# goodgodgd/xpt-mde-2021

Hardware: AMD Instinct MI355X
Metric: train images/sec (5-frame 128x416 snippets) (higher is better)
Workload: dtype bf16; 1 GPU; DepthNet(NASNetMobile)+PoseNetImproved train step, KITTI-raw-shaped 5x128x416 snippets, batch 8/GPU, mono L1+SSIM+smoothness, 4 scales; global_batch=8, per_gpu_batch=8, mode=graph, parallelism=dp1, ranks=1

## Files before the change

### include/xpt_hip.h

```cpp
#ifndef XPT_HIP_H_
#define XPT_HIP_H_

#include <stddef.h>
#include <stdint.h>

#ifdef __cplusplus
extern "C" {
#endif

#define XPT_OK 0
#define XPT_ERR_NULL (-1)
#define XPT_ERR_SHAPE (-2)
#define XPT_ERR_ARG (-3)
#define XPT_ERR_WORKSPACE (-4)
#define XPT_ERR_LAUNCH (-5)

#define XPT_PHOTO_L1 0
#define XPT_PHOTO_L2 1
#define XPT_PHOTO_SSIM 2

int xpt_abi_version(void);
const char* xpt_build_arch(void);

int xpt_pose_rvec2matr_fwd(const float* pose, float* T, int M, void* stream);
int xpt_pose_rvec2matr_bwd(const float* pose, const float* dT, float* dpose, int M, void* stream);

int xpt_resize_down_fwd(const float* img, float* out, int M, int H, int W, int C, int scale, void* stream);
int xpt_image_pyramids(const float* image5d, int B, int S, int H, int W, int njobs, const int* first_frame,
                       const int* nframes, const int* scale, float* const* out, void* stream);

int xpt_warp_fwd(const float* src, const float* depth, const float* T, const float* K, float* synth,
                 int B, int N, int h, int w, float scale, void* stream);
size_t xpt_warp_bwd_workspace_floats(int B, int N, int h, int w);
int xpt_warp_bwd(const float* src, const float* depth, const float* T, const float* K, const float* dsynth,
                 float* ddepth, float* dT, float* workspace, size_t workspace_floats,
                 int B, int N, int h, int w, float scale, void* stream);

int xpt_bilinear_fwd(const float* image, const float* coords, const float* valid_mask, float* out,
                     int B, int N, int h, int w, int C, int ncoord, void* stream);
int xpt_bilinear_bwd(const float* image, const float* coords, const float* valid_mask, const float* dout,
                     float* dcoords, int B, int N, int h, int w, int C, int ncoord, void* stream);

size_t xpt_photo_workspace_floats(int B, int N, int h, int w);
int xpt_photo_fwd(int method, const float* synth, const float* target, float* map, float* loss,
                  float* workspace, size_t workspace_floats, int B, int N, int h, int w, void* stream);
int xpt_photo_bwd(int method, const float* synth, const float* target, const float* gloss, const float* gmap,
                  float* dsynth, float* workspace, size_t workspace_floats, int B, int N, int h, int w,
                  void* stream);

int xpt_photo_fused_tune(int fwd_min_waves, int bwd_min_waves, int min_rows);
int xpt_photo_fused_variant(int pipelined);
size_t xpt_photo_fused_workspace_floats(int B, int N, int h, int w);
int xpt_photo_fused_fwd(const float* src, const float* depth, const float* T, const float* K, const float* target,
                        float* synth, float* loss_l1, float* loss_ssim, float* workspace, size_t workspace_floats,
                        int B, int N, int h, int w, float scale, void* stream);
int xpt_photo_fused_bwd(const float* src, const float* depth, const float* T, const float* K, const float* target,
                        const float* g_l1, const float* g_ssim, float* ddepth, float* dT, float* workspace,
                        size_t workspace_floats, int B, int N, int h, int w, float scale, void* stream);

int xpt_photo_fused_ms_fwd(int nscales, const float* const* src, const float* const* depth, const float* T, const float* K,
                           const float* const* target, float* losses, float* workspace, size_t workspace_floats,
                           int B, int N, const int* h, const int* w, const float* scale, void* stream);

int xpt_photo_fused_ms_bwd(int nscales, const float* const* src, const float* const* depth, const float* T, const float* K,
                           const float* const* target, const float* const* g_l1, const float* const* g_ssim,
                           float* const* ddepth, float* dT, float* workspace, size_t workspace_floats, int B, int N,
                           const int* h, const int* w, const float* scale, void* stream);

int xpt_photo_march_tune(int fwd_min_waves, int bwd_min_waves, int min_rows);
int xpt_photo_march_plan(int bwd_variant, int rows_s0, int rows_s1, int rows_s2, int rows_s3);
int xpt_photo_march_ms_fwd(int nscales, const float* const* src, const float* const* depth, const float* T, const float* K,
                           const float* const* target, float* losses, float* workspace, size_t workspace_floats,
                           int B, int N, const int* h, const int* w, const float* scale, void* stream);
int xpt_photo_march_ms_fwdbwd(int nscales, const float* const* src, const float* const* depth, const float* T, const float* K,
                              const float* const* target, const float* const* g_l1, const float* const* g_ssim,
                              float* losses, float* const* ddepth, float* dT, float* workspace, size_t workspace_floats,
                              int B, int N, const int* h, const int* w, const float* scale, void* stream);
int xpt_photo_march_ms_bwd(int nscales, const float* const* src, const float* const* depth, const float* T, const float* K,
                           const float* const* target, const float* const* g_l1, const float* const* g_ssim,
                           float* const* ddepth, float* dT, float* workspace, size_t workspace_floats, int B, int N,
                           const int* h, const int* w, const float* scale, void* stream);

size_t xpt_smooth_workspace_floats(int B, int h, int w);
int xpt_smooth_fwd(const float* disp, const float* image, float* loss, float* workspace, size_t workspace_floats,
                   int B, int h, int w, float grad_factor, int input_is_depth, void* stream);
int xpt_smooth_bwd(const float* disp, const float* image, const float* gloss, float* dinput,
                   int B, int h, int w, float grad_factor, int input_is_depth, void* stream);
int xpt_smooth_ms_fwd(int nscales, const float* const* disp, const float* const* image, float* losses,
                      float* workspace, size_t workspace_floats, int B, const int* h, const int* w, float grad_factor,
                      int input_is_depth, void* stream);
int xpt_smooth_ms_bwd(int nscales, const float* const* disp, const float* const* image, const float* const* gloss,
                      float* const* dinput, int B, const int* h, const int* w, float grad_factor, int input_is_depth,
                      void* stream);

int xpt_merge_total_fwd(int n, const float* const* terms, const float* c, const float* amat, float* total,
                        float* by_type, int batch, int types, void* stream);
int xpt_merge_total_bwd(int n, const float* c, const float* g_total, float* grads, int batch, void* stream);

int xpt_adam_step(float* param, float* grad, float* m, float* v, long long n, const float* step, float lr,
                  float beta1, float beta2, float eps, float grad_scale, int zero_grad, void* shadow_bf16,
                  void* stream);
int xpt_sgd_step(float* param, float* grad, long long n, float lr, float grad_scale, int zero_grad, void* shadow_bf16,
                 void* stream);

typedef struct xpt_loss_scale_state {
  float scale;
  float inv_scale;
  int found_inf;
  int good_steps;
  int skipped;
  int reserved[3];
} xpt_loss_scale_state;
int xpt_grad_nonfinite(const float* g, long long n, void* state, void* stream);
int xpt_loss_scale_update(void* state, int growth_steps, void* stream);
int xpt_adam_step_dyn(float* param, float* grad, float* m, float* v, long long n, const float* step, float lr,
                      float beta1, float beta2, float eps, float grad_scale, int zero_grad, void* shadow_bf16,
                      const void* state, void* stream);
int xpt_sgd_step_dyn(float* param, float* grad, long long n, float lr, float grad_scale, int zero_grad, void* shadow_bf16,
                     const void* state, void* stream);

int xpt_dwconv_fwd(const void* x, const float* w, void* y, int B, int H, int W, int C, int k, int stride, int pad_t,
                   int pad_l, int OH, int OW, int relu_in, int dtype, void* stream);
int xpt_dwconv_bwd_data(const void* x, const float* w, const void* dy, void* dx, int B, int H, int W, int C, int k,
                        int stride, int pad_t, int pad_l, int OH, int OW, int relu_in, int dtype, void* stream);
int xpt_dwconv_tune(int wrw_groups);
int xpt_set_xcd_affinity(int on);
int xpt_half_format(void);
size_t xpt_dwconv_bwd_weight_workspace_floats(int B, int OH, int OW, int C, int k);
int xpt_dwconv_bwd_weight(const void* x, const void* dy, float* dw, float* workspace, size_t workspace_floats,
                          int B, int H, int W, int C, int k, int stride, int pad_t, int pad_l, int OH, int OW,
                          int relu_in, int dtype, void* stream);

int xpt_affine_act_fwd(const void* x, const float* gamma, const float* beta, const float* mean, const float* var,
                       float eps, const void* residual, void* y, long long rows, int C, float slope, int relu_in,
                       int dtype, void* stream);
size_t xpt_affine_act_bwd_workspace_floats(long long rows, int C);
int xpt_affine_act_bwd(const void* x, const void* y, const void* dy, long long dy_pitch, const float* gamma,
                       const float* beta, const float* mean, const float* var, float eps, void* dx, float* dbeta,
                       float* dgamma, float* workspace, size_t workspace_floats, long long rows, int C, float slope,
                       int relu_in, int dtype, void* stream);

int xpt_conv1x1_bwd_weight_tune(int waves, int pairs_per_wave, int max_blocks, int max_partial_kib);
int xpt_conv1x1_bwd_weight_defer_cap(int mib);
size_t xpt_conv1x1_bwd_weight_workspace_floats(long long M, int cout, int cin);
int xpt_conv1x1_bwd_weight_counters(long long M, int cout, int cin);
int xpt_conv1x1_bwd_weight(const void* dy, const void* x, float* dw, float* workspace, size_t workspace_floats,
                           unsigned* counters, int n_counters, long long M, int cout, int cin, long long pitch_dy,
                           long long pitch_x, void* stream);

int xpt_pwconv_tune(int ksplit_min_cin, int ksplit_max_tiles);
int xpt_pwconv_bn_fwd(const void* x, const void* w, const float* gamma, const float* beta, const float* mean,
                      const float* var, float eps, const void* residual, void* ypre, void* y, long long M, int cin,
                      int cout, long long pitch_x, void* stream);

typedef struct xpt_conv_pack_job {
  const float* src;
  void* fwd;
  void* bwd;
  long long sn, sc, sh, sw;
  int N, T, KW, C, Cp, Np;
  long long first_block;
} xpt_conv_pack_job;
int xpt_conv_pack_job_bytes(void);
int xpt_conv_pack_weights(const void* jobs, int njobs, long long nblocks, void* stream);
int xpt_conv2d_tune(int plan);
int xpt_conv2d_fwd(const void* x, const void* w, const float* bias, void* y, int B, int PH, int PW, int C,
                   long long xpitch, int N, int KH, int KW, int stride, int pad_t, int pad_l, int OH, int OW,
                   long long ypitch, int upsample, float slope, void* stream);
int xpt_conv2d_bwd_data(const void* g, const void* wb, void* dx, int B, int OH, int OW, int Np, long long gpitch,
                        int C, int KH, int KW, int stride, int pad_t, int pad_l, int IH, int IW, long long dxpitch,
                        int fold2x2, void* stream);
int xpt_conv2d_splitk_tune(int enable, int force_split, int min_k, int max_pixels);
size_t xpt_conv2d_splitk_workspace_floats(long long pixels, int out_channels, int red_channels, int taps, int stride);
int xpt_conv2d_fwd_splitk(const void* x, const void* w, const float* bias, void* y, int B, int PH, int PW, int C,
                          long long xpitch, int N, int KH, int KW, int pad_t, int pad_l, int OH, int OW, long long ypitch,
                          int upsample, float slope, float* workspace, size_t workspace_floats, void* stream);
int xpt_conv2d_bwd_data_splitk(const void* g, const void* wb, void* dx, int B, int OH, int OW, int Np, long long gpitch,
                               int C, int KH, int KW, int pad_t, int pad_l, int IH, int IW, long long dxpitch, int fold2x2,
                               float* workspace, size_t workspace_floats, void* stream);
int xpt_conv2d_stream_tune(int enable, int min_tiles, int wgs_per_cu, int max_lds_kib);
int xpt_conv2d_stream_serves(int B, int OH, int OW, int out_channels, int red_channels, int KH, int KW, int stride,
                             int upsample_or_fold);
int xpt_conv2d_fwd_stream(const void* x, const void* w, const float* bias, void* y, int B, int PH, int PW, int C,
                          long long xpitch, int N, int pad_t, int pad_l, int OH, int OW, long long ypitch, int upsample,
                          float slope, void* stream);
int xpt_conv2d_fwd_stream_k5s2(const void* x, const void* w, const float* bias, void* y, int B, int PH, int PW, int C,
                               long long xpitch, int N, int pad_t, int pad_l, int OH, int OW, long long ypitch, float slope,
                               void* stream);
int xpt_conv2d_bwd_data_stream(const void* g, const void* wb, void* dx, int B, int OH, int OW, int Np, long long gpitch, int C,
                               int pad_t, int pad_l, int IH, int IW, long long dxpitch, int fold2x2, void* stream);
int xpt_conv2d_bwd_weight_tune(int max_partial_mib, int target_blocks);
int xpt_conv2d_bwd_weight_splits(int B, int C, int N, int KH, int KW, int stride, int OH, int OW);
int xpt_conv2d_bwd_weight_partials(const void* g, const void* x, float* partials, size_t partial_floats, int B, int PH,
                                   int PW, int C, int Cr, long long xpitch, int N, long long gpitch, int KH, int KW,
                                   int stride, int pad_t, int pad_l, int OH, int OW, int upsample, void* stream);
int xpt_restack_bf16(const float* image5d, void* out, int B, int S, int H, int W, int Cp, void* stream);

int xpt_headconv_tune(int passes, int max_blocks);
int xpt_headconv_bwd_blocks(int B, int H, int W, int C);
int xpt_headconv_fwd(const void* x, long long xpitch, const float* w, const float* bias, float* pre, int B, int H, int W,
                     int C, void* stream);
int xpt_headconv_bwd(const void* x, long long xpitch, const float* w, const float* g, void* dx, float* partials,
                     size_t partial_floats, int B, int H, int W, int C, void* stream);
int xpt_headconv_bwd_add(const void* x, long long xpitch, const float* w, const float* g, const void* addend,
                         long long addend_pitch, void* dx, float* partials, size_t partial_floats, int B, int H, int W, int C,
                         void* stream);

int xpt_depth_head_fwd(const float* x, float* depth, float* disp, long long n, void* stream);
int xpt_depth_head_bwd(const float* x, const float* g_depth, const float* g_disp, float* gx, long long n, void* stream);
int xpt_depth_head_ms_fwd(int nscales, const float* const* x, float* const* depth, float* const* disp, const long long* n,
                          void* stream);
int xpt_depth_head_ms_bwd(int nscales, const float* const* x, const float* const* g_depth, const float* const* g_disp,
                          float* const* gx, const long long* n, void* stream);

int xpt_global_avgpool_fwd(const void* x, float* y, int B, int HW, int C, int dtype, void* stream);
int xpt_global_avgpool_bwd(const float* g, void* dx, int B, int HW, int C, int dtype, void* stream);

int xpt_upsample2x_fwd(const float* src, void* out, long long M, int h, int w, int dtype, void* stream);
int xpt_upsample2x_bwd(const void* g, long long g_pitch, float* dsrc, long long M, int h, int w, int dtype, void* stream);
int xpt_upsample2x_bwd_add(const void* g, long long g_pitch, const float* addend, float* dsrc, long long M, int h, int w, int dtype,
                           void* stream);

int xpt_corr_cost_channels(int max_disp, int stride2);
int xpt_corr_cost_fwd(const void* left, const void* right, void* out, int B, int H, int W, int C, int max_disp,
                      int stride2, int dtype, void* stream);
int xpt_corr_cost_bwd(const void* left, const void* right, const void* gout, void* dleft, void* dright, int B, int H,
                      int W, int C, int max_disp, int stride2, int dtype, void* stream);

int xpt_avgpool3_same(const void* in, long long in_pitch, void* out, int B, int H, int W, int C, float scale, int adjoint,
                      int dtype, void* stream);

int xpt_pwconv_bn_multi_fwd(int n, const void* const* x, const void* const* w, const float* const* gamma,
                            const float* const* beta, const float* const* mean, const float* const* var, float eps,
                            const void* const* residual, void* const* ypre, void* const* y, long long M, int cin, int cout,
                            long long pitch_x, void* stream);
int xpt_pwconv_bn_multi_fwd_sib(int n, const void* const* x, const void* const* w, const float* const* gamma,
                                const float* const* beta, const float* const* mean, const float* const* var, float eps,
                                const void* const* residual, void* const* ypre, void* const* y, const void* const* sib_x,
                                const void* const* sib_w, const float* const* sib_gamma, const float* const* sib_beta,
                                const float* const* sib_mean, const float* const* sib_var, void* const* sib_ypre,
                                long long M, int cin, int cout, long long pitch_x, long long pitch_y, void* stream);

int xpt_multi_copy(const void* const* src, void* const* dst, const long long* bytes, int n, void* stream);

int xpt_concat_channels(const void* const* inputs, const long long* pitches, const int* channels, int n, void* out,
                        long long rows, int Ct, void* stream);

int xpt_sum_rows(const void* const* inputs, const long long* pitches, int n, void* out, long long rows, int C, int dtype,
                 void* stream);

int xpt_cell_tail_fwd(int nslices, const int* nterms, const void* const* src, const long long* pitch, const int* pooled,
                      const float* scale, void* out, long long out_pitch, int B, int H, int W, int F, int dtype,
                      void* stream);

int xpt_cell_tail_bwd(int ngrads, const void* const* grads, const long long* gpitch, const void* out, long long out_pitch,
                      void* gm, int nslices, int ndense, void* const* dense_out, const int* bterms, const int* slice,
                      const int* pooled, const float* scale, int B, int H, int W, int F, int dtype, void* stream);

int xpt_adjust_gather(const void* in, long long in_pitch, void* out, int B, int H, int W, int C, int dtype, void* stream);
int xpt_adjust_scatter(const void* d1, long long pitch1, const void* d2, long long pitch2, void* out, int B, int H, int W,
                       int C, int dtype, void* stream);

int xpt_pool_pair_fwd(const void* in, long long in_pitch, void* mp, void* ap, void* arg, int B, int H, int W, int C, int OH,
                      int OW, int pad_t, int pad_l, int dtype, void* stream);
int xpt_pool_pair_bwd(const void* gmp, long long pitch_m, const void* gap, long long pitch_a, const void* arg, void* dh, int B,
                      int H, int W, int C, int OH, int OW, int pad_t, int pad_l, int dtype, void* stream);
int xpt_pool_pair_bwd2(const void* gmp, long long pitch_m, const void* gmp2, long long pitch_m2, const void* gap, long long pitch_a,
                       const void* arg, void* dh, int B, int H, int W, int C, int OH, int OW, int pad_t, int pad_l, int dtype,
                       void* stream);

int xpt_augment(const float* u, float* params, const float* img0, float* img0_out, const float* img1, float* img1_out,
                int n_img, const float* depth, float* depth_out, int n_depth, const float* K0, float* K0_out, const float* K1,
                float* K1_out, int B, const float* pose0, float* pose0_out, const float* pose1, float* pose1_out, int n_pose,
                const float* stereo, float* stereo_out, int H, int W, float p_crop, float p_flip, float p_jit,
                float half_crop, void* stream);
int xpt_augment_pin(const float* pin);

int xpt_stem_input(const float* image, long long batch_stride, void* out, int B, int H, int W, void* stream);

int xpt_depth_metric(const float* pred, const float* gt, float* per_sample, int B, int h, int w, int r0, int r1, int c0,
                     int c1, float min_depth, float max_depth, void* stream);

int xpt_pose_metric(const float* pred, const float* truth, float* out, int B, int N, void* stream);

typedef struct xpt_reduce_job {
  float* dst;
  long long n;
  int nseg;
  int split_waves;
  const float* src[4];
  long long stride[4];
  int nsplit[4];
} xpt_reduce_job;
int xpt_reduce_job_bytes(void);
int xpt_reduce_partials(const void* jobs, const void* blockmap, int nblocks, void* stream);
int xpt_affine_act_bwd_blocks(long long rows, int C);
int xpt_affine_act_bwd_partials(const void* x, const void* y, const void* dy, long long dy_pitch, const float* gamma,
                                const float* beta, const float* mean, const float* var, float eps, void* dx,
                                float* partials, size_t partial_floats, long long rows, int C, float slope, int relu_in,
                                int dtype, void* stream);
int xpt_dwconv_bwd_weight_chunks(int B, int OH, int OW, int C, int k, int stride);
int xpt_dwconv_bwd_weight_partials(const void* x, const void* dy, float* partials, size_t partial_floats, int B, int H,
                                   int W, int C, int k, int stride, int pad_t, int pad_l, int OH, int OW, int relu_in,
                                   int dtype, void* stream);
int xpt_dwconv_bwd_both(const void* x, const float* w, const void* dy, void* dx, float* partials, size_t partial_floats,
                        int B, int H, int W, int C, int k, int stride, int pad_t, int pad_l, int OH, int OW, int relu_in,
                        int dtype, void* stream);
int xpt_conv1x1_bn_multi_bwd_partials(int n, const void* const* dy, const long long* pitch_dy, const void* const* ypre,
                                      const void* const* x, const float* const* gamma, const float* const* var,
                                      const float* const* mean, float eps, void* const* g_out, float* const* w_partials,
                                      float* const* bn_partials, size_t w_partial_floats, size_t bn_partial_floats,
                                      long long M, int cout, int cin, long long pitch_x, void* stream);
int xpt_conv1x1_bwd_fused(const void* dy, const void* x, const void* w, void* dx, float* partials,
                          size_t partial_floats, long long M, int cout, int cin, long long pitch_dy, long long pitch_x,
                          void* stream);
int xpt_conv1x1_bn_bwd_fused(const void* dy, const void* dy2, const void* dy3, const void* ypre, const void* x,
                             const void* w, const float* gamma, const float* var, const float* mean, float eps, void* dx,
                             float* w_partials, size_t w_partial_floats, float* bn_partials, size_t bn_partial_floats,
                             long long M, int cout, int cin, long long pitch_dy, long long pitch_dy2, long long pitch_dy3,
                             long long pitch_x, void* stream);
int xpt_conv1x1_bn_multi_bwd_fused(int n, const void* const* dy, const long long* pitch_dy, const void* const* ypre,
                                   const void* const* x, const void* const* w, const float* const* gamma,
                                   const float* const* var, const float* const* mean, float eps, void* const* dx,
                                   float* const* w_partials, float* const* bn_partials, size_t w_partial_floats,
                                   size_t bn_partial_floats, long long M, int cout, int cin, long long pitch_x,
                                   void* stream);
int xpt_conv1x1_bn_multi_bwd_fused_fan(int n, const void* const* dy, const long long* pitch_dy, const void* const* dy2,
                                       const long long* pitch_dy2, const void* const* dy3, const long long* pitch_dy3,
                                       const void* const* ypre, const void* const* x, const void* const* w,
                                       const float* const* gamma, const float* const* var, const float* const* mean,
                                       float eps, void* const* dx, float* const* w_partials, float* const* bn_partials,
                                       size_t w_partial_floats, size_t bn_partial_floats, long long M, int cout, int cin,
                                       long long pitch_x, void* stream);
int xpt_dwconv_multi_fwd(const void* const* x, const float* const* w, void* const* y, const int* k, const int* pad_t,
                         const int* pad_l, int n, int B, int H, int W, int C, int stride, int OH, int OW, int relu_in,
                         int dtype, void* stream);
int xpt_dwconv_multi_bwd(const void* const* xin, void* const* dxin, int n_inputs, const void* const* dy,
                         const float* const* w, float* const* partials, const int* k, const int* pad_t,
                         const int* pad_l, const int* input_of, int n, int B, int H, int W, int C, int stride, int OH,
                         int OW, int relu_in, int dtype, void* stream);
int xpt_conv1x1_bwd_weight_splits(long long M, int cout, int cin);
int xpt_conv1x1_bn_bwd_partials(const void* dy, const void* ypre, const void* x, const float* gamma, const float* var,
                                const float* mean, float eps, void* g_out, float* w_partials, size_t w_partial_floats,
                                float* bn_partials, size_t bn_partial_floats, long long M, int cout, int cin,
                                long long pitch_dy, long long pitch_x, void* stream);
int xpt_conv1x1_bn_bwd_partials_sum(const void* dy, const void* dy2, const void* dy3, const void* ypre, const void* x,
                                    const float* gamma, const float* var, const float* mean, float eps, void* g_out,
                                    float* w_partials, size_t w_partial_floats, float* bn_partials,
                                    size_t bn_partial_floats, long long M, int cout, int cin, long long pitch_dy,
                                    long long pitch_dy2, long long pitch_dy3, long long pitch_x, void* stream);
int xpt_conv1x1_bwd_weight_partials(const void* dy, const void* x, float* partials, size_t partial_floats, long long M,
                                    int cout, int cin, long long pitch_dy, long long pitch_x, void* stream);

uint32_t xpt_crc32c(const void* data, size_t nbytes);
long long xpt_tfrecord_index(const void* shard, size_t nbytes, int verify_crc, unsigned long long* payload_off,
                             unsigned long long* payload_len, unsigned int* payload_crc, long long max_records);
int xpt_tfrecord_decode(const void* payload, size_t nbytes, unsigned int stored_crc, int verify_crc, int nkeys,
                        const char* const* keys, void* const* dst, const size_t* dst_bytes);

int xpt_sepconv_bn_multi_fwd(int n, const void* const* x, const float* const* wdw, const void* const* wpw,
                             const float* const* gamma, const float* const* beta, const float* const* mean,
                             const float* const* var, const int* k, void* const* ydw, void* const* ypre,
                             const void* const* x_b, const float* const* wdw_b, const void* const* wpw_b,
                             const float* const* gamma_b, const float* const* beta_b, const float* const* mean_b,
                             const float* const* var_b, const int* k_b, void* const* ydw_b, void* const* ypre_b,
                             void* const* yb, const void* const* residual, void* const* y, float eps, int B, int H, int W,
                             int C, int cout, void* stream);

int xpt_dwconv_bn_relu6_fwd(const void* x, const float* w, const float* gamma, const float* beta, const float* mean,
                            const float* var, float eps, void* y, int B, int H, int W, int C, int stride, int pad_t, int pad_l,
                            int OH, int OW, int act_in, void* stream);
int xpt_dwconv_bn_relu6_tune(int fwd_outputs);
int xpt_dwconv_bn_relu6_fwd_outputs(int B, int OH, int OW, int C);
int xpt_dwconv_bn_relu6_bwd_chunks(int B, int OH, int OW, int C);
int xpt_dwconv_bn_relu6_bwd(const void* x, const void* y, const void* dy, long long dy_pitch, const float* w,
                            const float* gamma, const float* mean, const float* var, float eps, void* dx, float* partials,
                            size_t partial_floats, int B, int H, int W, int C, int stride, int pad_t, int pad_l, int OH, int OW,
                            int act_in, void* stream);

int xpt_graph_node_census(void* hip_graph, int* counts);

#ifdef __cplusplus
}
#endif
#endif
```

### xpt_mde_2021_amd/csrc/xpt_common.h

```cpp
#pragma once
#include <hip/hip_runtime.h>
#include <stdint.h>

#include "../../include/xpt_hip.h"

#define XPT_WAVE 64

#include <hip/hip_bf16.h>
#include <hip/hip_fp16.h>
#ifdef XPT_HALF_F16
typedef _Float16 xpt_h16;
typedef __half xpt_half_t;
#define XPT_MFMA_32X32X16(a, b, c) __builtin_amdgcn_mfma_f32_32x32x16_f16(a, b, c, 0, 0, 0)
#else
typedef __bf16 xpt_h16;
typedef __hip_bfloat16 xpt_half_t;
#define XPT_MFMA_32X32X16(a, b, c) __builtin_amdgcn_mfma_f32_32x32x16_bf16(a, b, c, 0, 0, 0)
#endif
typedef xpt_h16 xpt_h16x8 __attribute__((ext_vector_type(8)));
#ifdef __HIPCC__
__device__ __forceinline__ float xpt_h2f(unsigned short u) {
#ifdef XPT_HALF_F16
  return (float)__builtin_bit_cast(_Float16, u);
#else
  return __uint_as_float(((unsigned)u) << 16);
#endif
}
__device__ __forceinline__ float xpt_h2f_lo(unsigned w) {
#ifdef XPT_HALF_F16
  return (float)__builtin_bit_cast(_Float16, (unsigned short)(w & 0xffffu));
#else
  return __uint_as_float(w << 16);
#endif
}
__device__ __forceinline__ float xpt_h2f_hi(unsigned w) {
#ifdef XPT_HALF_F16
  return (float)__builtin_bit_cast(_Float16, (unsigned short)(w >> 16));
#else
  return __uint_as_float(w & 0xffff0000u);
#endif
}
__device__ __forceinline__ unsigned short xpt_f2h(float f) {
  return __builtin_bit_cast(unsigned short, (xpt_h16)f);
}
__device__ __forceinline__ unsigned short xpt_f2h_sw(float f) {
#ifdef XPT_HALF_F16
  return xpt_f2h(f);
#else
  unsigned u = __float_as_uint(f);
  u += 0x7fffu + ((u >> 16) & 1u);
  return (unsigned short)(u >> 16);
#endif
}
__device__ __forceinline__ float xpt_half2float(xpt_half_t h) {
#ifdef XPT_HALF_F16
  return __half2float(h);
#else
  return __bfloat162float(h);
#endif
}
__device__ __forceinline__ xpt_half_t xpt_float2half(float f) {
#ifdef XPT_HALF_F16
  return __float2half(f);
#else
  return __float2bfloat16(f);
#endif
}
#endif

#define XPT_CHECK_PTR(p) \
  do {                   \
    if ((p) == nullptr) return XPT_ERR_NULL; \
  } while (0)

static inline int xpt_launch_status() { return hipGetLastError() == hipSuccess ? XPT_OK : XPT_ERR_LAUNCH; }
#define XPT_BEGIN_LAUNCH() (void)hipGetLastError()

__device__ __forceinline__ unsigned xpt_divmod(unsigned n, unsigned d, unsigned& rem) {
  const float inv = __builtin_amdgcn_rcpf((float)d);
  unsigned q = (unsigned)((float)n * inv);
  int r = (int)(n - q * d);
  q += (unsigned)(int)((float)r * inv);
  r = (int)(n - q * d);
  if (r < 0) { --q; r += (int)d; }
  if (r < 0) { --q; r += (int)d; }
  if (r >= (int)d) { ++q; r -= (int)d; }
  if (r >= (int)d) { ++q; r -= (int)d; }
  rem = (unsigned)r;
  return q;
}
__device__ __forceinline__ void xpt_split4(unsigned idx, int n0, int n1, int n2, int& i0, int& i1, int& i2, int& i3) {
  unsigned r0, r1, r2;
  unsigned q = xpt_divmod(idx, (unsigned)n0, r0);
  q = xpt_divmod(q, (unsigned)n1, r1);
  q = xpt_divmod(q, (unsigned)n2, r2);
  i0 = (int)r0; i1 = (int)r1; i2 = (int)r2; i3 = (int)q;
}

namespace xpt {

struct Cam {
  float k[9];
  float ki[9];
};

__device__ inline Cam load_cam(const float* __restrict__ K, float scale) {
  Cam c;
#pragma unroll
  for (int i = 0; i < 6; ++i) c.k[i] = K[i] / scale;
  c.k[6] = 0.f;
  c.k[7] = 0.f;
  c.k[8] = 1.f;
  const float a = c.k[0], b = c.k[1], cc = c.k[2], d = c.k[3], e = c.k[4], f = c.k[5], g = c.k[6], h = c.k[7],
              i = c.k[8];
  const float A = e * i - f * h, Bc = -(d * i - f * g), Cc = d * h - e * g;
  const float det = a * A + b * Bc + cc * Cc;
  const float r = 1.0f / det;
  c.ki[0] = A * r;
  c.ki[1] = -(b * i - cc * h) * r;
  c.ki[2] = (b * f - cc * e) * r;
  c.ki[3] = Bc * r;
  c.ki[4] = (a * i - cc * g) * r;
  c.ki[5] = -(a * f - cc * d) * r;
  c.ki[6] = Cc * r;
  c.ki[7] = -(a * h - b * g) * r;
  c.ki[8] = (a * e - b * d) * r;
  return c;
}

struct Pose {
  float r[9];
  float t[3];
};

__device__ inline Pose load_pose(const float* __restrict__ T) {
  Pose p;
#pragma unroll
  for (int i = 0; i < 3; ++i) {
    p.r[3 * i + 0] = T[4 * i + 0];
    p.r[3 * i + 1] = T[4 * i + 1];
    p.r[3 * i + 2] = T[4 * i + 2];
    p.t[i] = T[4 * i + 3];
  }
  return p;
}

struct Warp {
  float X[3];
  float ray[3];
  float up, vp;
  float zinv;
};

__device__ inline void backproject(const Cam& c, float u, float v, float d, Warp& w) {
#pragma unroll
  for (int i = 0; i < 3; ++i) {
    w.ray[i] = c.ki[3 * i + 0] * u + c.ki[3 * i + 1] * v + c.ki[3 * i + 2];
    w.X[i] = w.ray[i] * d;
  }
}

__device__ inline void project(const Cam& c, const Pose& p, Warp& w) {
  float Xs[3], q[3];
#pragma unroll
  for (int i = 0; i < 3; ++i) Xs[i] = p.r[3 * i + 0] * w.X[0] + p.r[3 * i + 1] * w.X[1] + p.r[3 * i + 2] * w.X[2] + p.t[i];
#pragma unroll
  for (int i = 0; i < 3; ++i) q[i] = c.k[3 * i + 0] * Xs[0] + c.k[3 * i + 1] * Xs[1] + c.k[3 * i + 2] * Xs[2];
  const float z = q[2] + 1e-10f;
  w.zinv = 1.0f / z;
  w.up = q[0] / z;
  w.vp = q[1] / z;
}

struct Taps {
  int uf, uc, vf, vc;
  float wuf, wuc, wvf, wvc;
  float mask;
};

__device__ inline float clampf(float x, float lo, float hi) { return fminf(fmaxf(x, lo), hi); }

__device__ inline Taps make_taps(float u, float v, int h, int w, bool extra_valid) {
  Taps t;
  const float fu = floorf(u), fv = floorf(v);
  const float ufc = clampf(fu, 0.f, (float)(w - 1));
  const float ucc = clampf(fu + 1.f, 0.f, (float)(w - 1));
  const float vfc = clampf(fv, 0.f, (float)(h - 1));
  const float vcc = clampf(fv + 1.f, 0.f, (float)(h - 1));
  const bool ok = (ufc + 1.f == ucc) && (vfc + 1.f == vcc) && extra_valid;
  t.mask = ok ? 1.f : 0.f;
  t.uf = ok ? (int)ufc : 0;
  t.uc = ok ? (int)ucc : 0;
  t.vf = ok ? (int)vfc : 0;
  t.vc = ok ? (int)vcc : 0;
  t.wuf = ok ? (ucc - u) : 0.f;
  t.wuc = ok ? (u - ufc) : 0.f;
  t.wvf = ok ? (vcc - v) : 0.f;
  t.wvc = ok ? (v - vfc) : 0.f;
  return t;
}

__device__ inline float wave_sum(float v) {
#pragma unroll
  for (int off = 32; off > 0; off >>= 1) v += __shfl_down(v, off, 64);
  return v;
}

__device__ inline float block_sum(float v, float* red) {
  const int lane = threadIdx.x & 63, wid = threadIdx.x >> 6, nw = (blockDim.x + 63) >> 6;
  v = wave_sum(v);
  __syncthreads();
  if (lane == 0) red[wid] = v;
  __syncthreads();
  float s = 0.f;
  if (threadIdx.x == 0) {
    for (int i = 0; i < nw; ++i) s += red[i];
  }
  return s;
}

template <int NV>
__device__ inline void block_sum_n(float (&v)[NV], float* red) {
  const int lane = threadIdx.x & 63, wid = threadIdx.x >> 6, nw = (blockDim.x + 63) >> 6;
#pragma unroll
  for (int i = 0; i < NV; ++i) v[i] = wave_sum(v[i]);
  __syncthreads();
  if (lane == 0) {
#pragma unroll
    for (int i = 0; i < NV; ++i) red[wid * NV + i] = v[i];
  }
  __syncthreads();
  if (threadIdx.x == 0) {
#pragma unroll
    for (int i = 0; i < NV; ++i) {
      float s = 0.f;
      for (int k = 0; k < nw; ++k) s += red[k * NV + i];
      v[i] = s;
    }
  }
}

}

extern int g_xpt_xcd_affinity;
#ifdef __HIPCC__
__device__ __forceinline__ void xpt_xcd_remap(bool on, unsigned& bx, unsigned& by, unsigned gx, unsigned gy) {
  if (!on) return;
  const unsigned lin = bx + gx * by, total = gx * gy;
  const unsigned u = (lin & 7u) * (total >> 3) + (lin >> 3);
  by = u / gx;
  bx = u - by * gx;
}
#endif
inline bool xpt_xcd_ok(unsigned long long total) { return g_xpt_xcd_affinity != 0 && total % 8 == 0 && total >= 64; }

inline unsigned xpt_xcd_pad(unsigned long long n) { return (unsigned)((n + 7) & ~7ull); }
inline unsigned xpt_magic(unsigned d) { return d <= 1 ? 0u : (unsigned)((0x100000000ull + d - 1) / d); }
#ifdef __HIPCC__
__device__ __forceinline__ unsigned xpt_fastdiv(unsigned n, unsigned m) { return m ? __umulhi(n, m) : n; }
#endif

struct XcdSweep {
  unsigned grid, units, per;
  int on;
#ifdef __HIPCC__
  __device__ __forceinline__ bool range(unsigned x, long long total, long long& begin, long long& end) const;
#endif
};
inline XcdSweep xpt_xcd_sweep(long long total, long long max_units, int threads = 256) {
  XcdSweep s;
  long long units = (total + threads - 1) / threads;
  if (units > max_units) units = max_units;
  if (units < 1) units = 1;
  s.per = (unsigned)(((total + units - 1) / units + threads - 1) / threads * threads);
  s.units = (unsigned)((total + s.per - 1) / s.per);
  if (s.units < 1) s.units = 1;
  s.on = g_xpt_xcd_affinity;
  s.grid = s.on ? xpt_xcd_pad(s.units) : s.units;
  return s;
}
#ifdef __HIPCC__
__device__ __forceinline__ bool xpt_xcd_unit(bool on, unsigned x, unsigned n, unsigned& u) {
  if (!on) {
    u = x;
    return x < n;
  }
  const unsigned k = x & 7u, q = x >> 3;
  const unsigned lo = (k * n) >> 3, hi = ((k + 1u) * n) >> 3;
  u = lo + q;
  return u < hi;
}
inline unsigned xpt_xcd_two_class_grid(int on, unsigned nA, unsigned LA, unsigned nB, unsigned LB) {
  return on ? nA * xpt_xcd_pad(LA) + nB * xpt_xcd_pad(LB) : nA * LA + nB * LB;
}
__device__ __forceinline__ bool xpt_xcd_two_class(bool on, unsigned x, unsigned nA, unsigned LA, unsigned nB, unsigned LB,
                                                  unsigned& vb) {
  if (!on) {
    vb = x;
    return true;
  }
  const unsigned a8 = nA * ((LA + 7u) & ~7u);
  const bool first = x < a8;
  const unsigned L = first ? LA : LB, lin = first ? x : x - a8;
  const unsigned c8 = (L + 7u) >> 3, k = lin & 7u, q = lin >> 3;
  unsigned local;
  const unsigned seg = xpt_divmod(q, c8, local);
  const unsigned lo = (k * L) >> 3, hi = ((k + 1u) * L) >> 3;
  vb = (first ? 0u : nA * LA) + seg * L + lo + local;
  return lo + local < hi;
}
__device__ __forceinline__ void xpt_chunk_range(unsigned blk, unsigned nblocks, long long total, long long& begin, long long& end) {
  unsigned rem_;
  const unsigned per = (xpt_divmod((unsigned)total + nblocks - 1u, nblocks, rem_) + 255u) & ~255u;
  begin = (long long)blk * per;
  end = begin + per < total ? begin + per : total;
}
__device__ __forceinline__ bool XcdSweep::range(unsigned x, long long total, long long& begin, long long& end) const {
  unsigned u;
  if (!xpt_xcd_unit(on != 0, x, units, u)) return false;
  begin = (long long)u * per;
  end = begin + per < total ? begin + per : total;
  return true;
}
#endif
```

### xpt_mde_2021_amd/csrc/xpt_conv_wgrad.hip

```cpp
#include "xpt_common.h"

namespace {

typedef float f32x16 __attribute__((ext_vector_type(16)));
typedef xpt_h16x8 bf16x8;
typedef short s16x4 __attribute__((ext_vector_type(4)));
typedef short s16x8 __attribute__((ext_vector_type(8)));
typedef unsigned int u32x4 __attribute__((ext_vector_type(4)));

constexpr int WGRAD_MAXCH = 12;

struct WgradArgs {
  const unsigned short* g;
  const unsigned short* x;
  float* part;
  long long gpitch, xpitch, gbytes, xbytes;
  int B, PH, PW, shift, Hlim, Wlim;
  int C, Cr, N, KH, KW, stride, pad_t, pad_l, OH, OW;
  int R, CB, nseg, nrb, units, nsplit;
  int WN, WC, WT;
  int dbg;
};

__device__ inline bf16x8 tr_pair(const char* lds, unsigned off0, unsigned off1) {
  typedef s16x4 __attribute__((address_space(3))) * lds_ptr;
  const s16x4 lo = __builtin_amdgcn_ds_read_tr16_b64_v4i16((lds_ptr)(lds + off0));
  const s16x4 hi = __builtin_amdgcn_ds_read_tr16_b64_v4i16((lds_ptr)(lds + off1));
  s16x8 v;
  v[0] = lo[0]; v[1] = lo[1]; v[2] = lo[2]; v[3] = lo[3];
  v[4] = hi[0]; v[5] = hi[1]; v[6] = hi[2]; v[7] = hi[3];
  return __builtin_bit_cast(bf16x8, v);
}

template <int MAXCH>
struct WgradChunks {
  int row[MAXCH], col[MAXCH];
  unsigned chb[MAXCH];
};

constexpr unsigned WG_OOB = 0x40000000u;

template <int MAXCH>
__device__ __forceinline__ void wgrad_chunks(const WgradArgs& a, int tid, int n0, int c0, int TNB, int TCB, int Wt,
                                             int gi, int gchunks, int xchunks, WgradChunks<MAXCH>& w) {
  const int lg = __builtin_ctz((unsigned)(TNB >> 3)), lx = __builtin_ctz((unsigned)(TCB >> 3));
  const float inv_cb = 1.f / (float)a.CB, inv_wt = 1.f / (float)Wt;
#pragma unroll
  for (int i = 0; i < MAXCH; ++i) {
    if (i < gi) {
      const int ck = tid + 256 * i;
      const int gc8 = ck & ((1 << lg) - 1), gpix = ck >> lg;
      const int gr = (int)(((float)gpix + 0.5f) * inv_cb);
      w.row[i] = gr;
      w.col[i] = gpix - gr * a.CB;
      const int n = n0 + 8 * gc8;
      w.chb[i] = (ck < gchunks && n < a.N) ? (unsigned)n * 2u : WG_OOB;
    } else {
      const int cx = tid + 256 * (i - gi);
      const int xc8 = cx & ((1 << lx) - 1), xpix = cx >> lx;
      const int xr = (int)(((float)xpix + 0.5f) * inv_wt);
      w.row[i] = xr;
      w.col[i] = xpix - xr * Wt;
      const int c = c0 + 8 * xc8;
      w.chb[i] = (cx < xchunks && c < a.C) ? (unsigned)c * 2u : WG_OOB;
    }
  }
}

template <int MAXCH>
__device__ __forceinline__ void wgrad_fetch(const WgradArgs& a, int u, int gi, const WgradChunks<MAXCH>& w,
                                            const __amdgpu_buffer_rsrc_t& rg, const __amdgpu_buffer_rsrc_t& rx, u32x4 (&stage)[MAXCH]) {
  unsigned seg, rb;
  const unsigned q1 = xpt_divmod((unsigned)u, (unsigned)a.nseg, seg);
  const unsigned b = xpt_divmod(q1, (unsigned)a.nrb, rb);
  const int oh0 = (int)rb * a.R, ow0 = (int)seg * a.CB;
  const int th0 = oh0 * a.stride - a.pad_t, tw0 = ow0 * a.stride - a.pad_l;
  const unsigned gimg = b * (unsigned)(a.OH * a.OW), ximg = b * (unsigned)(a.PH * a.PW);
  const unsigned gp2 = (unsigned)(a.gpitch * 2), xp2 = (unsigned)(a.xpitch * 2);
#pragma unroll
  for (int i = 0; i < MAXCH; ++i) {
    if (i < gi) {
      const int r = oh0 + w.row[i], c = ow0 + w.col[i];
      const bool ok = r < a.OH && c < a.OW;
      const unsigned off = ok ? (gimg + (unsigned)(r * a.OW + c)) * gp2 + w.chb[i] : WG_OOB;
      stage[i] = __builtin_amdgcn_raw_buffer_load_b128(rg, off, 0, 0);
    } else {
      const int r = th0 + w.row[i], c = tw0 + w.col[i];
      const bool ok = r >= 0 && c >= 0 && r < a.Hlim && c < a.Wlim;
      const unsigned off = ok ? (ximg + (unsigned)((r >> a.shift) * a.PW + (c >> a.shift))) * xp2 + w.chb[i] : WG_OOB;
      stage[i] = __builtin_amdgcn_raw_buffer_load_b128(rx, off, 0, 0);
    }
  }
}

template <int TAPS>
__global__ __launch_bounds__(256) void conv_wgrad_kernel(WgradArgs a) {
  extern __shared__ __attribute__((aligned(16))) char smem[];
  const int tid = threadIdx.x, lane = tid & 63, wave = tid >> 6;
  const int TNB = 32 * a.WN, TCB = 32 * a.WC;
  const int T = a.KH * a.KW;
  const int ntc = (a.C + TCB - 1) / TCB;
  const int n0 = (blockIdx.x / ntc) * TNB, c0 = (blockIdx.x % ntc) * TCB;
  const int HR = (a.R - 1) * a.stride + a.KH, Wt = (a.CB - 1) * a.stride + a.KW;
  const int gchunks = a.R * a.CB * (TNB / 8), xchunks = HR * Wt * (TCB / 8);
  const int gi = (gchunks + 255) >> 8;
  char* gs = smem;
  char* xs = smem + (size_t)gi * 256 * 16;

  const int wt = wave % a.WT, wc = (wave / a.WT) % a.WC, wn = wave / (a.WT * a.WC);
  const int tap0 = wt * TAPS;
  const bool active = tap0 < T;
  const int g4 = lane >> 4, li = lane & 15, q = li >> 2, p = li & 3, h = g4 >> 1, half = g4 & 1;
  unsigned a_base[2], b_base[2];
#pragma unroll
  for (int i = 0; i < 2; ++i) {
    const int pc = 8 * h + 4 * i + q;
    a_base[i] = (unsigned)((pc * TNB + wn * 32 + 16 * half + 4 * p) * 2);
    b_base[i] = (unsigned)((pc * a.stride * TCB + wc * 32 + 16 * half + 4 * p) * 2);
  }
  unsigned toff[TAPS];
#pragma unroll
  for (int t = 0; t < TAPS; ++t) {
    const int tap = tap0 + t < T ? tap0 + t : 0;
    toff[t] = (unsigned)(((tap / a.KW) * Wt + (tap % a.KW)) * TCB * 2);
  }

  f32x16 acc[TAPS];
#pragma unroll
  for (int t = 0; t < TAPS; ++t)
#pragma unroll
    for (int e = 0; e < 16; ++e) acc[t][e] = 0.f;

  constexpr int MAXCH = WGRAD_MAXCH;
  const __amdgpu_buffer_rsrc_t rg = __builtin_amdgcn_make_buffer_rsrc((void*)a.g, 0, (int)a.gbytes, 0x00020000);
  const __amdgpu_buffer_rsrc_t rx = __builtin_amdgcn_make_buffer_rsrc((void*)a.x, 0, (int)a.xbytes, 0x00020000);
  u32x4 stage[MAXCH];
  WgradChunks<MAXCH> chunks;
  wgrad_chunks<MAXCH>(a, tid, n0, c0, TNB, TCB, Wt, gi, gchunks, xchunks, chunks);
  int u = blockIdx.y;
  if (u < a.units) wgrad_fetch<MAXCH>(a, u, gi, chunks, rg, rx, stage);
  for (; u < a.units; u += a.nsplit) {
    __syncthreads();
#pragma unroll
    for (int i = 0; i < MAXCH; ++i) {
      const int ck = tid + 256 * i;
      if (i < gi ? ck < gchunks : ck - gi * 256 < xchunks) *(u32x4*)(smem + (size_t)ck * 16) = stage[i];
    }
    __syncthreads();
    if (u + a.nsplit < a.units && !(a.dbg & 2))
      wgrad_fetch<MAXCH>(a, u + a.nsplit, gi, chunks, rg, rx, stage);
    if (active && !(a.dbg & 1)) {
      for (int rr = 0; rr < a.R; ++rr) {
        for (int c16 = 0; c16 < a.CB; c16 += 16) {
          const unsigned ga = (unsigned)((rr * a.CB + c16) * TNB * 2);
          const unsigned xa = (unsigned)(((rr * a.stride) * Wt + c16 * a.stride) * TCB * 2);
          const bf16x8 fa = tr_pair(gs, a_base[0] + ga, a_base[1] + ga);
#pragma unroll
          for (int t = 0; t < TAPS; ++t) {
            if (tap0 + t < T) {
              const bf16x8 fb = tr_pair(xs, b_base[0] + xa + toff[t], b_base[1] + xa + toff[t]);
              acc[t] = XPT_MFMA_32X32X16(fa, fb, acc[t]);
            }
          }
        }
      }
    }
  }

  if (!active || (a.dbg & 4)) return;
  const int c = c0 + wc * 32 + (lane & 31);
  float* dst = a.part + (long long)blockIdx.y * a.N * T * a.Cr;
#pragma unroll
  for (int t = 0; t < TAPS; ++t) {
    if (tap0 + t >= T) continue;
#pragma unroll
    for (int e = 0; e < 16; ++e) {
      const int n = n0 + wn * 32 + (e & 3) + 8 * (e >> 2) + 4 * h;
      if (n < a.N && c < a.Cr) dst[((long long)n * T + tap0 + t) * a.Cr + c] = acc[t][e];
    }
  }
}

struct WfArgs {
  const unsigned short* g;
  const unsigned short* x;
  float* part;
  long long gpitch, xpitch, gbytes, xbytes;
  int B, PH, PW, OH, OW, C, Cr, N;
  int pad_t, pad_l, taps;
  int tiles_x, tiles_y, ntiles, nsplit, ct, nb;
  int xcd;
};

template <int K, int S, bool UPS>
__global__ __launch_bounds__(256) void conv_wgrad_fast_kernel(WfArgs a) {
  constexpr int HR = UPS ? 6 : 7 * S + K, WR = UPS ? 10 : 15 * S + K, HPIX = HR * WR;
  constexpr int T = K * K, TPW = (T + 3) / 4;
  __shared__ __attribute__((aligned(16))) char smem[8192 + HPIX * 64];
  constexpr int NG = 2, NX = (HPIX * 4 + 255) / 256;
  char* const gs = smem;
  char* const xs = smem + 8192;
  const int tid = threadIdx.x, lane = tid & 63, wave = __builtin_amdgcn_readfirstlane((int)(threadIdx.x >> 6));
  int cblk, nblk, split;
  if (a.xcd) {
    unsigned sp_, cb_;
    const unsigned rest = xpt_divmod(blockIdx.x, (unsigned)a.nsplit, sp_);
    nblk = (int)xpt_divmod(rest, (unsigned)a.ct, cb_);
    cblk = (int)cb_;
    split = (int)sp_;
  } else {
    cblk = (int)blockIdx.x % a.ct;
    nblk = ((int)blockIdx.x / a.ct) % a.nb;
    split = (int)blockIdx.x / (a.ct * a.nb);
  }
  const int c0 = cblk * 32, n0 = nblk * 32;
  const __amdgpu_buffer_rsrc_t rg = __builtin_amdgcn_make_buffer_rsrc((void*)a.g, 0, (int)a.gbytes, 0x00020000);
  const __amdgpu_buffer_rsrc_t rx = __builtin_amdgcn_make_buffer_rsrc((void*)a.x, 0, (int)a.xbytes, 0x00020000);
  const unsigned gp2 = (unsigned)(a.gpitch * 2), xp2 = (unsigned)(a.xpitch * 2);

  int grow[NG], gcol[NG];
  unsigned gcb[NG], gconst[NG];
#pragma unroll
  for (int i = 0; i < NG; ++i) {
    const int v = tid + 256 * i, pix = v >> 2, cv = v & 3;
    grow[i] = pix >> 4;
    gcol[i] = pix & 15;
    gcb[i] = n0 + cv * 8 < a.N ? (unsigned)(n0 + cv * 8) * 2u : WG_OOB;
    gconst[i] = (unsigned)(grow[i] * a.OW + gcol[i]) * gp2 + gcb[i];
  }
  int xq[NX], xrem[NX], xlds[NX];
  unsigned xcb[NX], xconst[NX];
#pragma unroll
  for (int i = 0; i < NX; ++i) {
    const int v = tid + 256 * i, pix = v >> 2, cv = v & 3;
    const int q = pix / WR, rem = pix - q * WR;
    const bool live = pix < HPIX;
    xq[i] = q;
    xrem[i] = rem;
    xlds[i] = live ? pix * 64 + cv * 16 : -1;
    xcb[i] = (live && c0 + cv * 8 < a.C) ? (unsigned)(c0 + cv * 8) * 2u : WG_OOB;
    xconst[i] = (unsigned)(q * a.PW + rem) * xp2 + xcb[i];
  }

  const int g4 = lane >> 4, li = lane & 15, q4 = li >> 2, p4 = li & 3, h = g4 >> 1, half = g4 & 1;
  unsigned abase[2];
  int tkh[TPW];
  unsigned bsel[TPW][2];
#pragma unroll
  for (int i = 0; i < 2; ++i) abase[i] = (unsigned)((8 * h + 4 * i + q4) * 64 + (16 * half + 4 * p4) * 2);
#pragma unroll
  for (int tt = 0; tt < TPW; ++tt) {
    const int tap = wave + 4 * tt;
    const int kh = tap / K, kw = tap - K * kh;
    tkh[tt] = tap < T ? kh : -1;
#pragma unroll
    for (int i = 0; i < 2; ++i) {
      const int pc = 8 * h + 4 * i + q4;
      const int col = UPS ? ((pc + kw - 1) >> 1) + 1 : pc * S + kw;
      bsel[tt][i] = (unsigned)(8192 + col * 64 + (16 * half + 4 * p4) * 2);
    }
  }
  f32x16 acc[TPW];
#pragma unroll
  for (int t = 0; t < TPW; ++t)
#pragma unroll
    for (int e = 0; e < 16; ++e) acc[t][e] = 0.f;

  auto tile_of = [&](int t, int& b, int& oh0, int& ow0) {
    unsigned u = (unsigned)t;
    if (a.xcd) u = (u & 7u) * ((unsigned)a.ntiles >> 3) + (u >> 3);
    unsigned txi, tyi;
    const unsigned q1 = xpt_divmod(u, (unsigned)a.tiles_x, txi);
    b = __builtin_amdgcn_readfirstlane((int)xpt_divmod(q1, (unsigned)a.tiles_y, tyi));
    oh0 = __builtin_amdgcn_readfirstlane((int)tyi * 8);
    ow0 = __builtin_amdgcn_readfirstlane((int)txi * 16);
  };
  u32x4 sg[NG], sx[NX];
  auto fetch = [&](int t) {
    int b, oh0, ow0;
    tile_of(t, b, oh0, ow0);
    const int plo_h = UPS ? (oh0 - 1) >> 1 : oh0 * S - a.pad_t, plo_w = UPS ? (ow0 - 1) >> 1 : ow0 * S - a.pad_l;
    const bool g_in = oh0 + 8 <= a.OH && ow0 + 16 <= a.OW;
    const bool x_in = plo_h >= 0 && plo_h + HR <= a.PH && plo_w >= 0 && plo_w + WR <= a.PW;
    if (g_in) {
      const unsigned soff = (unsigned)((b * a.OH + oh0) * a.OW + ow0) * gp2;
#pragma unroll
      for (int i = 0; i < NG; ++i) sg[i] = __builtin_amdgcn_raw_buffer_load_b128(rg, gconst[i], soff, 0);
    } else {
#pragma unroll
      for (int i = 0; i < NG; ++i) {
        const int r = oh0 + grow[i], c = ow0 + gcol[i];
        const unsigned off = (r < a.OH && c < a.OW) ? (unsigned)((b * a.OH + r) * a.OW + c) * gp2 + gcb[i] : WG_OOB;
        sg[i] = __builtin_amdgcn_raw_buffer_load_b128(rg, off, 0, 0);
      }
    }
    if (x_in) {
      const unsigned soff = (unsigned)((b * a.PH + plo_h) * a.PW + plo_w) * xp2;
#pragma unroll
      for (int i = 0; i < NX; ++i) sx[i] = __builtin_amdgcn_raw_buffer_load_b128(rx, xconst[i], soff, 0);
    } else {
#pragma unroll
      for (int i = 0; i < NX; ++i) {
        const int pr = plo_h + xq[i], pc = plo_w + xrem[i];
        const bool ok = (unsigned)pr < (unsigned)a.PH && (unsigned)pc < (unsigned)a.PW;
        const unsigned off = ok ? (unsigned)((b * a.PH + pr) * a.PW + pc) * xp2 + xcb[i] : WG_OOB;
        sx[i] = __builtin_amdgcn_raw_buffer_load_b128(rx, off, 0, 0);
      }
    }
  };

  int t = split;
  if (t < a.ntiles) fetch(t);
  for (; t < a.ntiles; t += a.nsplit) {
    __syncthreads();
#pragma unroll
    for (int i = 0; i < NG; ++i) *(u32x4*)(gs + (tid + 256 * i) * 16) = sg[i];
#pragma unroll
    for (int i = 0; i < NX; ++i)
      if (xlds[i] >= 0) *(u32x4*)(xs + xlds[i]) = sx[i];
    __syncthreads();
    if (t + a.nsplit < a.ntiles) fetch(t + a.nsplit);
#pragma unroll
    for (int rr = 0; rr < 8; ++rr) {
      const bf16x8 fa = tr_pair(smem, abase[0] + rr * 1024, abase[1] + rr * 1024);
#pragma unroll
      for (int tt = 0; tt < TPW; ++tt) {
        if (tkh[tt] >= 0) {
          const int hrow = UPS ? ((rr + tkh[tt] - 1) >> 1) + 1 : rr * S + tkh[tt];
          const unsigned ro = (unsigned)(hrow * WR * 64);
          const bf16x8 fb = tr_pair(smem, bsel[tt][0] + ro, bsel[tt][1] + ro);
          acc[tt] = XPT_MFMA_32X32X16(fa, fb, acc[tt]);
        }
      }
    }
  }

  const int c = c0 + (lane & 31);
  float* dst = a.part + (long long)split * a.N * T * a.Cr;
#pragma unroll
  for (int tt = 0; tt < TPW; ++tt) {
    const int tap = wave + 4 * tt;
    if (tap >= T) continue;
#pragma unroll
    for (int e = 0; e < 16; ++e) {
      const int n = n0 + (e & 3) + 8 * (e >> 2) + 4 * h;
      if (n < a.N && c < a.Cr) dst[((long long)n * T + tap) * a.Cr + c] = acc[tt][e];
    }
  }
}

int g_wgrad_fast = 1;
int g_wgrad_fast_min_tiles = 1;

bool fast_plan(int B, int C, int N, int KH, int KW, int stride, int OH, int OW, int upsample, WfArgs& a) {
  if (!g_wgrad_fast || KH != KW || !((KH == 3 && (stride == 1 || stride == 2)) || (KH == 5 && stride == 2))) return false;
  if (upsample && (KH != 3 || stride != 1)) return false;
  (void)upsample;
  a.tiles_x = (OW + 15) / 16;
  a.tiles_y = (OH + 7) / 8;
  const long long nt = (long long)B * a.tiles_y * a.tiles_x;
  if (nt < g_wgrad_fast_min_tiles || nt > 0x3fffffffLL) return false;
  a.ntiles = (int)nt;
  a.ct = (C + 31) / 32;
  a.nb = (N + 31) / 32;
  a.taps = KH * KW;
  return true;
}

struct WgradPlan {
  int WN, WC, WT, TAPS, R, CB, nseg, nrb, units, nsplit;
  long long blocks;
  size_t lds;
};


int g_wgrad_max_partial_mib = 12, g_wgrad_target_blocks = 512, g_wgrad_dbg = 0;

int fast_nsplit(const WfArgs& a, int N, int C) {
  const long long bytes = (long long)N * a.taps * C * 4;
  long long s = (768 + a.ct * a.nb - 1) / (a.ct * a.nb);
  const long long cap = ((long long)g_wgrad_max_partial_mib << 20) / (bytes > 0 ? bytes : 1);
  if (s > cap) s = cap;
  if (s > a.ntiles) s = a.ntiles;
  if (s >= 16) s &= ~7ll;
  return s < 1 ? 1 : (int)s;
}


bool plan_for(int wn, int wc, int B, int C, int N, int KH, int KW, int stride, int OH, int OW, WgradPlan& p) {
  const int T = KH * KW;
  p.WN = wn; p.WC = wc;
  p.WT = 4 / (wn * wc);
  const int taps = (T + p.WT - 1) / p.WT;
  const int allowed[] = {1, 3, 5, 7, 9};
  p.TAPS = 0;
  for (int v : allowed)
    if (v >= taps) { p.TAPS = v; break; }
  if (!p.TAPS) return false;
  const int TNB = 32 * wn, TCB = 32 * wc;
  const size_t max_lds = (size_t)WGRAD_MAXCH * 256 * 16;
  const int ow16 = (OW + 15) / 16 * 16;
  p.CB = ow16 < 64 ? ow16 : 64;
  p.nseg = (OW + p.CB - 1) / p.CB;
  p.R = 256 / p.CB;
  if (p.R < 1) p.R = 1;
  if (p.R > OH) p.R = OH;
  for (;;) {
    const int HR = (p.R - 1) * stride + KH, Wt = (p.CB - 1) * stride + KW;
    const size_t gch = (size_t)p.R * p.CB * (TNB / 8), xch = (size_t)HR * Wt * (TCB / 8);
    const size_t slots = (gch + 255) / 256 + (xch + 255) / 256;
    p.lds = ((gch + 255) / 256 * 256 + xch) * 16;
    if (slots <= (size_t)WGRAD_MAXCH && p.lds <= max_lds) break;
    if (p.R > 1) p.R -= 1;
    else if (p.CB > 16) { p.CB -= 16; p.nseg = (OW + p.CB - 1) / p.CB; }
    else return false;
  }
  p.nrb = (OH + p.R - 1) / p.R;
  p.units = B * p.nrb * p.nseg;
  const long long tiles = (long long)((N + TNB - 1) / TNB) * ((C + TCB - 1) / TCB);
  long long ns = (g_wgrad_target_blocks + tiles - 1) / tiles;
  const long long bytes = (long long)N * T * C * 4;
  const long long cap = ((long long)g_wgrad_max_partial_mib << 20) / (bytes > 0 ? bytes : 1);
  if (ns > cap) ns = cap;
  if (ns > p.units) ns = p.units;
  if (ns < 1) ns = 1;
  p.nsplit = (int)ns;
  p.blocks = tiles * ns;
  return true;
}

bool make_plan(int B, int C, int N, int KH, int KW, int stride, int OH, int OW, WgradPlan& best) {
  const int cand[4][2] = {{2, 2}, {2, 1}, {1, 2}, {1, 1}};
  bool have = false;
  for (const auto& wc : cand) {
    if ((wc[0] == 2 && N <= 32) || (wc[1] == 2 && C <= 32)) continue;
    if (KH * KW > 9 && wc[0] * wc[1] > 1) continue;
    WgradPlan p;
    if (!plan_for(wc[0], wc[1], B, C, N, KH, KW, stride, OH, OW, p)) continue;
    if (!have || p.blocks > best.blocks) { best = p; have = true; }
    if (best.blocks * 4 >= (long long)g_wgrad_target_blocks * 3) break;
  }
  return have;
}

}

extern "C" int xpt_conv2d_bwd_weight_tune(int max_partial_mib, int target_blocks) {
  if (max_partial_mib == -1000) {
    g_wgrad_fast = target_blocks != 0;
    g_wgrad_fast_min_tiles = target_blocks > 1 ? target_blocks : 1;
    return XPT_OK;
  }
  if (max_partial_mib < 0) g_wgrad_dbg = -max_partial_mib;
  if (max_partial_mib > 0) g_wgrad_max_partial_mib = max_partial_mib;
  if (target_blocks > 0) g_wgrad_target_blocks = target_blocks;
  return XPT_OK;
}

extern "C" int xpt_conv2d_bwd_weight_splits(int B, int C, int N, int KH, int KW, int stride, int OH, int OW) {
  WgradPlan p;
  if (B <= 0 || C <= 0 || N <= 0 || KH <= 0 || KW <= 0 || stride <= 0 || OH <= 0 || OW <= 0) return XPT_ERR_SHAPE;
  WfArgs f{};
  if (fast_plan(B, C, N, KH, KW, stride, OH, OW, 0, f)) return fast_nsplit(f, N, C);
  if (!make_plan(B, C, N, KH, KW, stride, OH, OW, p)) return XPT_ERR_ARG;
  return p.nsplit;
}

extern "C" int xpt_conv2d_bwd_weight_partials(const void* g, const void* x, float* partials, size_t partial_floats, int B,
                                              int PH, int PW, int C, int Cr, long long xpitch, int N, long long gpitch,
                                              int KH, int KW, int stride, int pad_t, int pad_l, int OH, int OW,
                                              int upsample, void* stream) {
  XPT_CHECK_PTR(g); XPT_CHECK_PTR(x); XPT_CHECK_PTR(partials);
  if (B <= 0 || PH <= 0 || PW <= 0 || C <= 0 || Cr <= 0 || Cr > C || N <= 0 || KH <= 0 || KW <= 0 || OH <= 0 || OW <= 0)
    return XPT_ERR_SHAPE;
  if (C % 8 != 0 || N % 8 != 0 || xpitch < C || xpitch % 8 != 0 || gpitch < N || gpitch % 8 != 0 ||
      ((uintptr_t)g) % 16 != 0 || ((uintptr_t)x) % 16 != 0 || stride < 1 || (upsample != 0 && upsample != 1))
    return XPT_ERR_ARG;
  {
    WfArgs f{};
    if (fast_plan(B, C, N, KH, KW, stride, OH, OW, upsample, f) &&
        (upsample ? ((long long)PH * 2 == OH && (long long)PW * 2 == OW && pad_t == 1 && pad_l == 1)
                  : ((long long)(OH - 1) * stride - pad_t < PH && (long long)(OW - 1) * stride - pad_l < PW))) {
      f.nsplit = fast_nsplit(f, N, C);
      if (partial_floats < (size_t)f.nsplit * N * KH * KW * Cr) return XPT_ERR_WORKSPACE;
      f.g = (const unsigned short*)g; f.x = (const unsigned short*)x; f.part = partials;
      f.gpitch = gpitch; f.xpitch = xpitch;
      f.gbytes = ((long long)B * OH * OW - 1) * gpitch * 2 + (long long)N * 2;
      f.xbytes = ((long long)B * PH * PW - 1) * xpitch * 2 + (long long)C * 2;
      if (f.gbytes >= (1LL << 30) || f.xbytes >= (1LL << 30)) return XPT_ERR_SHAPE;
      f.B = B; f.PH = PH; f.PW = PW; f.OH = OH; f.OW = OW; f.C = C; f.Cr = Cr; f.N = N; f.pad_t = pad_t; f.pad_l = pad_l;
      f.xcd = (g_xpt_xcd_affinity != 0 && f.ntiles % 8 == 0 && f.nsplit % 8 == 0) ? 1 : 0;
      const dim3 grid(f.ct * f.nb * f.nsplit);
      hipStream_t st = (hipStream_t)stream;
      XPT_BEGIN_LAUNCH();
      if (upsample) hipLaunchKernelGGL((conv_wgrad_fast_kernel<3, 1, true>), grid, dim3(256), 0, st, f);
      else if (KH == 3 && stride == 1) hipLaunchKernelGGL((conv_wgrad_fast_kernel<3, 1, false>), grid, dim3(256), 0, st, f);
      else if (KH == 3) hipLaunchKernelGGL((conv_wgrad_fast_kernel<3, 2, false>), grid, dim3(256), 0, st, f);
      else hipLaunchKernelGGL((conv_wgrad_fast_kernel<5, 2, false>), grid, dim3(256), 0, st, f);
      return xpt_launch_status();
    }
  }
  WgradPlan p;
  if (!make_plan(B, C, N, KH, KW, stride, OH, OW, p)) return XPT_ERR_ARG;
  if (partial_floats < (size_t)p.nsplit * N * KH * KW * Cr) return XPT_ERR_WORKSPACE;
  WgradArgs a{};
  a.g = (const unsigned short*)g; a.x = (const unsigned short*)x; a.part = partials;
  a.gpitch = gpitch; a.xpitch = xpitch;
  a.gbytes = ((long long)B * OH * OW - 1) * gpitch * 2 + (long long)N * 2;
  a.xbytes = ((long long)B * PH * PW - 1) * xpitch * 2 + (long long)C * 2;
  if (a.gbytes >= (1LL << 30) || a.xbytes >= (1LL << 30)) return XPT_ERR_SHAPE;
  a.B = B; a.PH = PH; a.PW = PW; a.shift = upsample; a.Hlim = PH << upsample; a.Wlim = PW << upsample;
  a.C = C; a.Cr = Cr; a.N = N; a.KH = KH; a.KW = KW; a.stride = stride; a.pad_t = pad_t; a.pad_l = pad_l;
  a.OH = OH; a.OW = OW;
  a.R = p.R; a.CB = p.CB; a.nseg = p.nseg; a.nrb = p.nrb; a.units = p.units; a.nsplit = p.nsplit;
  a.WN = p.WN; a.WC = p.WC; a.WT = p.WT;
  a.dbg = g_wgrad_dbg;
  const int TNB = 32 * p.WN, TCB = 32 * p.WC;
  const dim3 grid(((N + TNB - 1) / TNB) * ((C + TCB - 1) / TCB), p.nsplit);
  hipStream_t s = (hipStream_t)stream;
  XPT_BEGIN_LAUNCH();
#define XPT_WGRAD_CASE(TP)                                                                                         \
  case TP: {                                                                                                       \
    hipLaunchKernelGGL(conv_wgrad_kernel<TP>, grid, dim3(256), p.lds, s, a);                                       \
  } break;
  switch (p.TAPS) {
    XPT_WGRAD_CASE(1)
    XPT_WGRAD_CASE(3)
    XPT_WGRAD_CASE(5)
    XPT_WGRAD_CASE(7)
    XPT_WGRAD_CASE(9)
    default:
      return XPT_ERR_ARG;
  }
#undef XPT_WGRAD_CASE
  return xpt_launch_status();
}
```

### xpt_mde_2021_amd/csrc/xpt_pointwise.hip

```cpp

#include "xpt_common.h"

namespace {

template <typename T> __device__ inline float ldf(const T* p);
template <> __device__ inline float ldf<float>(const float* p) { return *p; }
template <> __device__ inline float ldf<xpt_half_t>(const xpt_half_t* p) { return xpt_half2float(*p); }
template <typename T> __device__ inline void stf(T* p, float v);
template <> __device__ inline void stf<float>(float* p, float v) { *p = v; }
template <> __device__ inline void stf<xpt_half_t>(xpt_half_t* p, float v) { *p = xpt_float2half(v); }

struct Affine {
  const float* gamma;
  const float* beta;
  const float* mean;
  const float* var;
  float eps;
};

__device__ inline void affine_coeffs(const Affine& a, int c, float& sc, float& sh, float& rstd, float& mu) {
  if (a.gamma) {
    rstd = rsqrtf(a.var[c] + a.eps);
    mu = a.mean[c];
    sc = a.gamma[c] * rstd;
    sh = a.beta[c] - mu * sc;
  } else {
    rstd = 1.f; mu = 0.f; sc = 1.f; sh = a.beta[c];
  }
}

template <typename T>
__global__ void affine_act_fwd_kernel(const T* __restrict__ x, Affine a, const T* __restrict__ residual,
                                      T* __restrict__ y, long long n, int C, float slope, int relu_in, XcdSweep sw) {
  long long i, i_end;
  if (!sw.range(blockIdx.x, n, i, i_end)) return;
  for (i += threadIdx.x; i < i_end; i += 256) {
    unsigned c_;
    (void)xpt_divmod((unsigned)i, (unsigned)C, c_);
    const int c = (int)c_;
    float sc, sh, rstd, mu;
    affine_coeffs(a, c, sc, sh, rstd, mu);
    float v = ldf<T>(x + i);
    if (relu_in) v = fmaxf(v, 0.f);
    v = v * sc + sh;
    v = v > 0.f ? v : v * slope;
    if (residual) v += ldf<T>(residual + i);
    stf<T>(y + i, v);
  }
}

template <typename T, int V> struct RowVec;
template <> struct RowVec<float, 4> { typedef float4 type; };
template <> struct RowVec<float, 2> { typedef float2 type; };
template <> struct RowVec<float, 1> { typedef float type; };
template <> struct RowVec<xpt_half_t, 8> { typedef uint4 type; };
template <> struct RowVec<xpt_half_t, 4> { typedef uint2 type; };
template <> struct RowVec<xpt_half_t, 2> { typedef unsigned type; };
template <> struct RowVec<xpt_half_t, 1> { typedef unsigned short type; };

template <typename T, int V>
__device__ inline void load_row(const T* p, float (&out)[V]) {
  typename RowVec<T, V>::type raw = *(const typename RowVec<T, V>::type*)p;
  const T* e = (const T*)&raw;
#pragma unroll
  for (int i = 0; i < V; ++i) out[i] = ldf<T>(e + i);
}

template <typename T, int V>
__device__ inline void store_row(T* p, const float (&v)[V]) {
  typename RowVec<T, V>::type raw;
  T* e = (T*)&raw;
#pragma unroll
  for (int i = 0; i < V; ++i) stf<T>(e + i, v[i]);
  *(typename RowVec<T, V>::type*)p = raw;
}

#define PW_MAX_GROUPS 64
template <typename T, int V>
__global__ __launch_bounds__(256) void affine_act_bwd_kernel(const T* __restrict__ x, const T* __restrict__ y,
                                                              const T* __restrict__ dy, long long dy_pitch, Affine a,
                                                              T* __restrict__ dx, float* __restrict__ part,
                                                              long long rows, int C, long long rows_per_block,
                                                              float slope, int relu_in, int need_dscale,
                                                              int final_partials, int nblocks, int xcd) {
  __shared__ float red[2][256 * V];
  unsigned rb;
  if (!xpt_xcd_unit(xcd != 0, blockIdx.x, (unsigned)nblocks, rb)) return;
  const int groups = C / V;
  const int g0 = blockIdx.y * PW_MAX_GROUPS;
  const int gt = min(groups - g0, PW_MAX_GROUPS);
  const int slots = 256 / gt;
  const int grp = threadIdx.x % gt, slot = threadIdx.x / gt;
  const int c0 = (g0 + grp) * V;
  const long long r_begin = (long long)rb * rows_per_block;
  const long long r_end = min(rows, r_begin + rows_per_block);
  float s_shift[V], s_scale[V], sc[V];
#pragma unroll
  for (int i = 0; i < V; ++i) s_shift[i] = s_scale[i] = 0.f;
  if (slot < slots) {
#pragma unroll
    for (int i = 0; i < V; ++i) {
      float sh, rstd, mu;
      affine_coeffs(a, c0 + i, sc[i], sh, rstd, mu);
    }
#pragma unroll 2
    for (long long r = r_begin + slot; r < r_end; r += slots) {
      const long long o = r * C + c0;
      float g[V], xv[V], gx[V];
      load_row<T, V>(dy + r * dy_pitch + c0, g);
      if (slope != 1.f) {
        float yv[V];
        load_row<T, V>(y + o, yv);
#pragma unroll
        for (int i = 0; i < V; ++i) g[i] = yv[i] > 0.f ? g[i] : g[i] * slope;
      }
      if (need_dscale || relu_in) {
        load_row<T, V>(x + o, xv);
      } else {
#pragma unroll
        for (int i = 0; i < V; ++i) xv[i] = 0.f;
      }
#pragma unroll
      for (int i = 0; i < V; ++i) {
        gx[i] = g[i] * sc[i];
        if (relu_in) {
          if (!(xv[i] > 0.f)) gx[i] = 0.f;
          xv[i] = fmaxf(xv[i], 0.f);
        }
        s_shift[i] += g[i];
        s_scale[i] += g[i] * xv[i];
      }
      if (dx) store_row<T, V>(dx + o, gx);
    }
  }
  const int width = gt * V;
  if (slot < slots) {
#pragma unroll
    for (int i = 0; i < V; ++i) {
      red[0][slot * width + grp * V + i] = s_shift[i];
      red[1][slot * width + grp * V + i] = s_scale[i];
    }
  }
  __syncthreads();
  for (int e = threadIdx.x; e < width; e += 256) {
    float s0 = 0.f, s1 = 0.f;
    for (int k = 0; k < slots; ++k) {
      s0 += red[0][k * width + e];
      s1 += red[1][k * width + e];
    }
    const int c = g0 * V + e;
    if (final_partials && need_dscale) {
      float scc, sh, rstd, mu;
      affine_coeffs(a, c, scc, sh, rstd, mu);
      s1 = rstd * (s1 - mu * s0);
    }
    float* p = part + (long long)rb * 2 * C;
    p[c] = s0;
    p[C + c] = s1;
  }
}

struct SumInputs {
  const void* ptr[8];
  long long pitch[8];
  int n;
};

template <typename T, int V>
__global__ __launch_bounds__(256) void sum_rows_kernel(SumInputs in, T* __restrict__ out, long long rows, int C, XcdSweep sw) {
  const int groups = C / V;
  const long long total = rows * groups;
  long long idx, idx_end;
  if (!sw.range(blockIdx.x, total, idx, idx_end)) return;
  for (idx += threadIdx.x; idx < idx_end; idx += 256) {
    unsigned c0_;
    const long long r = (long long)xpt_divmod((unsigned)idx, (unsigned)groups, c0_);
    const int c0 = (int)c0_ * V;
    float acc[V], v[7][V];
    load_row<T, V>((const T*)in.ptr[0] + r * in.pitch[0] + c0, acc);
#pragma unroll
    for (int i = 1; i < 8; ++i) {
      const int k = i < in.n ? i : 0;
      load_row<T, V>((const T*)in.ptr[k] + r * in.pitch[k] + c0, v[i - 1]);
    }
#pragma unroll
    for (int i = 1; i < 8; ++i)
#pragma unroll
      for (int j = 0; j < V; ++j) acc[j] += i < in.n ? v[i - 1][j] : 0.f;
    store_row<T, V>(out + r * C + c0, acc);
  }
}

struct CopyJobs {
  const unsigned char* src[8];
  unsigned char* dst[8];
  long long first[9];
  long long bytes[8];
  int n;
};

__global__ __launch_bounds__(256) void multi_copy_kernel(CopyJobs jobs) {
  const long long total = jobs.first[jobs.n];
  for (long long v = blockIdx.x * 256LL + threadIdx.x; v < total; v += gridDim.x * 256LL) {
    int j = 0;
#pragma unroll
    for (int i = 1; i < 8; ++i)
      if (i < jobs.n && v >= jobs.first[i]) j = i;
    const long long off = (v - jobs.first[j]) * 16;
    if (off + 16 <= jobs.bytes[j] && ((((uintptr_t)jobs.src[j]) | ((uintptr_t)jobs.dst[j])) & 15) == 0) {
      *(uint4*)(jobs.dst[j] + off) = *(const uint4*)(jobs.src[j] + off);
    } else {
      for (long long b = off; b < off + 16 && b < jobs.bytes[j]; ++b) jobs.dst[j][b] = jobs.src[j][b];
    }
  }
}

struct CatInputs {
  const unsigned short* ptr[4];
  long long pitch[4];
  int first[5];
  int n;
};

__global__ __launch_bounds__(256) void concat_channels_kernel(CatInputs in, unsigned short* __restrict__ out, unsigned total,
                                                              int groups, XcdSweep sw) {
  long long i64, e64;
  if (!sw.range(blockIdx.x, (long long)total, i64, e64)) return;
  for (unsigned idx = (unsigned)i64 + threadIdx.x; idx < (unsigned)e64; idx += 256u) {
    unsigned g_;
    const long long row = (long long)xpt_divmod(idx, (unsigned)groups, g_);
    const int c0 = (int)g_ * 8;
    uint4 val = make_uint4(0u, 0u, 0u, 0u);
    bool done = false;
#pragma unroll
    for (int i = 0; i < 4; ++i) {
      if (i < in.n && c0 >= in.first[i] && c0 + 8 <= in.first[i + 1]) {
        const unsigned short* src = in.ptr[i] + row * in.pitch[i] + (c0 - in.first[i]);
        if (((uintptr_t)src & 15) == 0) {
          val = *(const uint4*)src;
          done = true;
        }
      }
    }
    if (!done) {
      unsigned short e[8];
#pragma unroll
      for (int k = 0; k < 8; ++k) {
        const int c = c0 + k;
        unsigned short v = 0;
#pragma unroll
        for (int i = 0; i < 4; ++i)
          if (i < in.n && c >= in.first[i] && c < in.first[i + 1]) v = in.ptr[i][row * in.pitch[i] + (c - in.first[i])];
        e[k] = v;
      }
      val.x = e[0] | ((unsigned)e[1] << 16); val.y = e[2] | ((unsigned)e[3] << 16);
      val.z = e[4] | ((unsigned)e[5] << 16); val.w = e[6] | ((unsigned)e[7] << 16);
    }
    *(uint4*)(out + (row * groups + (long long)g_) * 8) = val;
  }
}

template <typename T, int V>
__global__ __launch_bounds__(256) void avgpool3_kernel(const T* __restrict__ in, long long in_pitch, T* __restrict__ out,
                                                       int B, int H, int W, int C, float scale, int adjoint) {
  const int groups = C / V;
  const long long total = (long long)B * H * W * groups;
  for (long long idx = blockIdx.x * (long long)blockDim.x + threadIdx.x; idx < total;
       idx += (long long)gridDim.x * blockDim.x) {
    unsigned c0_;
    long long p = (long long)xpt_divmod((unsigned)idx, (unsigned)groups, c0_);
    const int c0 = (int)c0_ * V;
    unsigned r1_, r2_;
    const unsigned q1_ = xpt_divmod((unsigned)p, (unsigned)W, r1_);
    const int b = (int)xpt_divmod(q1_, (unsigned)H, r2_);
    const int x = (int)r1_, y = (int)r2_;
    float acc[V];
#pragma unroll
    for (int j = 0; j < V; ++j) acc[j] = 0.f;
#pragma unroll
    for (int dy = -1; dy <= 1; ++dy) {
#pragma unroll
      for (int dx = -1; dx <= 1; ++dx) {
        const int ny = y + dy, nx = x + dx;
        const bool ok = ny >= 0 && ny < H && nx >= 0 && nx < W;
        const int cy = min(max(ny, 0), H - 1), cx = min(max(nx, 0), W - 1);
        float v[V];
        load_row<T, V>(in + (((long long)b * H + cy) * W + cx) * in_pitch + c0, v);
        float wgt = ok ? 1.f : 0.f;
        if (adjoint) {
          const int cnt = ((cy > 0) + 1 + (cy < H - 1)) * ((cx > 0) + 1 + (cx < W - 1));
          wgt = ok ? 1.f / (float)cnt : 0.f;
        }
#pragma unroll
        for (int j = 0; j < V; ++j) acc[j] += v[j] * wgt;
      }
    }
    float norm = scale;
    if (!adjoint) norm = scale / (float)(((y > 0) + 1 + (y < H - 1)) * ((x > 0) + 1 + (x < W - 1)));
#pragma unroll
    for (int j = 0; j < V; ++j) acc[j] *= norm;
    store_row<T, V>(out + (((long long)b * H + y) * W + x) * C + c0, acc);
  }
}

__global__ void depth_head_fwd_kernel(const float* __restrict__ x, float* __restrict__ depth, float* __restrict__ disp,
                                      long long n) {
  for (long long i = blockIdx.x * (long long)blockDim.x + threadIdx.x; i < n; i += (long long)gridDim.x * blockDim.x) {
    const float sg = 1.f / (1.f + expf(-x[i]));
    const float u = sg + 0.01f;
    const float d = u > 1e-5f ? 1.f / u : 0.f;
    depth[i] = d;
    disp[i] = d > 1e-5f ? 1.f / d : 0.f;
  }
}

__global__ void depth_head_bwd_kernel(const float* __restrict__ x, const float* __restrict__ g_depth,
                                      const float* __restrict__ g_disp, float* __restrict__ gx, long long n) {
  for (long long i = blockIdx.x * (long long)blockDim.x + threadIdx.x; i < n; i += (long long)gridDim.x * blockDim.x) {
    const float sg = 1.f / (1.f + expf(-x[i]));
    const float u = sg + 0.01f;
    const float d = u > 1e-5f ? 1.f / u : 0.f;
    float gd = g_depth ? g_depth[i] : 0.f;
    if (g_disp && d > 1e-5f) gd -= g_disp[i] / (d * d);
    const float gu = u > 1e-5f ? -gd / (u * u) : 0.f;
    gx[i] = gu * sg * (1.f - sg);
  }
}

template <typename T>
__global__ void gap_fwd_kernel(const T* __restrict__ x, float* __restrict__ y, int total, int HW, int C) {
  const int i = blockIdx.x * blockDim.x + threadIdx.x;
  if (i >= total) return;
  const int b = i / C, c = i - b * C;
  const T* p = x + (long long)b * HW * C + c;
  float s = 0.f;
  for (int k = 0; k < HW; ++k) s += ldf<T>(p + (long long)k * C);
  y[i] = s / (float)HW;
}

template <typename T>
__global__ void gap_bwd_kernel(const float* __restrict__ g, T* __restrict__ dx, long long total, int HW, int C) {
  for (long long i = blockIdx.x * (long long)blockDim.x + threadIdx.x; i < total; i += (long long)gridDim.x * blockDim.x) {
    unsigned c_;
    (void)xpt_divmod((unsigned)i, (unsigned)C, c_);
    const int c = (int)c_;
    const long long b = i / ((long long)HW * C);
    stf<T>(dx + i, g[b * C + c] / (float)HW);
  }
}

__device__ inline void up2_taps(int y, int h, int& i0, int& i1, float& l) {
  const float src = fmaxf(0.5f * (float)y - 0.25f, 0.f);
  i0 = (int)src;
  i1 = min(i0 + 1, h - 1);
  l = src - (float)i0;
}

template <typename T>
__global__ void upsample2x_fwd_kernel(const float* __restrict__ src, T* __restrict__ out, long long total, int h, int w,
                                      XcdSweep sw) {
  const int H = 2 * h, W = 2 * w;
  long long i, i_end;
  if (!sw.range(blockIdx.x, total, i, i_end)) return;
  for (i += threadIdx.x; i < i_end; i += 256) {
    unsigned xu, yu;
    const long long m = (long long)xpt_divmod(xpt_divmod((unsigned)i, (unsigned)W, xu), (unsigned)H, yu);
    const int x = (int)xu, y = (int)yu;
    int y0, y1, x0, x1;
    float ly, lx;
    up2_taps(y, h, y0, y1, ly);
    up2_taps(x, w, x0, x1, lx);
    const float* p = src + m * h * w;
    const float top = (1.f - lx) * p[(long long)y0 * w + x0] + lx * p[(long long)y0 * w + x1];
    const float bot = (1.f - lx) * p[(long long)y1 * w + x0] + lx * p[(long long)y1 * w + x1];
    stf<T>(out + i, (1.f - ly) * top + ly * bot);
  }
}

__device__ inline float up2_weight(int y, int i, int h) {
  if (y < 0 || y >= 2 * h) return 0.f;
  int i0, i1;
  float l;
  up2_taps(y, h, i0, i1, l);
  return (i0 == i ? 1.f - l : 0.f) + (i1 == i ? l : 0.f);
}

template <typename T>
__global__ void upsample2x_bwd_kernel(const T* __restrict__ g, long long g_pitch, const float* __restrict__ addend,
                                      float* __restrict__ dsrc, long long total, int h, int w, XcdSweep sw) {
  const int W = 2 * w, H = 2 * h;
  long long idx, idx_end;
  if (!sw.range(blockIdx.x, total, idx, idx_end)) return;
  for (idx += threadIdx.x; idx < idx_end; idx += 256) {
    unsigned ju, iu;
    const long long m = (long long)xpt_divmod(xpt_divmod((unsigned)idx, (unsigned)w, ju), (unsigned)h, iu);
    const int j = (int)ju, i = (int)iu;
    const T* gm = g + m * H * W * g_pitch;
    float acc = 0.f;
#pragma unroll
    for (int dy = -1; dy <= 2; ++dy) {
      const int y = 2 * i + dy;
      const float wy = up2_weight(y, i, h);
      if (wy == 0.f) continue;
      float row = 0.f;
#pragma unroll
      for (int dx = -1; dx <= 2; ++dx) {
        const int x = 2 * j + dx;
        const float wx = up2_weight(x, j, w);
        if (wx != 0.f) row += wx * ldf<T>(gm + ((long long)y * W + x) * g_pitch);
      }
      acc += wy * row;
    }
    dsrc[idx] = addend != nullptr ? addend[idx] + acc : acc;
  }
}

struct DepthHeadMs {
  const float* x[4];
  float* depth[4];
  float* disp[4];
  const float* g_depth[4];
  const float* g_disp[4];
  long long n[4];
};

__global__ void depth_head_ms_fwd_kernel(DepthHeadMs a) {
  const int s = blockIdx.y;
  const float* __restrict__ x = a.x[s];
  float* __restrict__ depth = a.depth[s];
  float* __restrict__ disp = a.disp[s];
  const long long n = a.n[s];
  for (long long i = blockIdx.x * (long long)blockDim.x + threadIdx.x; i < n; i += (long long)gridDim.x * blockDim.x) {
    const float sg = 1.f / (1.f + expf(-x[i]));
    const float u = sg + 0.01f;
    const float d = u > 1e-5f ? 1.f / u : 0.f;
    depth[i] = d;
    disp[i] = d > 1e-5f ? 1.f / d : 0.f;
  }
}

__global__ void depth_head_ms_bwd_kernel(DepthHeadMs a) {
  const int s = blockIdx.y;
  const float* __restrict__ x = a.x[s];
  const float* __restrict__ g_depth = a.g_depth[s];
  const float* __restrict__ g_disp = a.g_disp[s];
  float* __restrict__ gx = a.depth[s];
  const long long n = a.n[s];
  for (long long i = blockIdx.x * (long long)blockDim.x + threadIdx.x; i < n; i += (long long)gridDim.x * blockDim.x) {
    const float sg = 1.f / (1.f + expf(-x[i]));
    const float u = sg + 0.01f;
    const float d = u > 1e-5f ? 1.f / u : 0.f;
    float gd = g_depth ? g_depth[i] : 0.f;
    if (g_disp && d > 1e-5f) gd -= g_disp[i] / (d * d);
    const float gu = u > 1e-5f ? -gd / (u * u) : 0.f;
    gx[i] = gu * sg * (1.f - sg);
  }
}

__global__ void affine_finish_kernel(const float* __restrict__ part, Affine a, float* __restrict__ dbeta,
                                     float* __restrict__ dgamma, int C, int nblk) {
  const int c = blockIdx.x * 4 + (threadIdx.x >> 6);
  const int t = threadIdx.x & 63;
  float s0 = 0.f, s1 = 0.f;
  if (c < C)
    for (int k = t; k < nblk; k += 64) {
      s0 += part[(long long)k * 2 * C + c];
      s1 += part[(long long)k * 2 * C + C + c];
    }
#pragma unroll
  for (int off = 32; off > 0; off >>= 1) {
    s0 += __shfl_down(s0, off, 64);
    s1 += __shfl_down(s1, off, 64);
  }
  if (t == 0 && c < C) {
    dbeta[c] = s0;
    if (dgamma) {
      float sc, sh, rstd, mu;
      affine_coeffs(a, c, sc, sh, rstd, mu);
      dgamma[c] = rstd * (s1 - mu * s0);
    }
  }
}

inline unsigned grid_for(long long total) {
  long long blocks = (total + 255) / 256;
  if (blocks > 4096) blocks = 4096;
  if (blocks < 1) blocks = 1;
  return (unsigned)blocks;
}

static long long affine_bwd_rows_per_block(long long rows) {
  long long rpb = (rows + 511) / 512;
  if (rpb < 8) rpb = 8;
  return (rpb + 7) / 8 * 8;
}

static int affine_bwd_blocks(long long rows, int C) {
  const long long rpb = affine_bwd_rows_per_block(rows);
  return (int)((rows + rpb - 1) / rpb);
}

template <typename T, int V>
static void affine_bwd_launch_v(const void* x, const void* y, const void* dy, long long dy_pitch, const Affine& a,
                                void* dx, float* part, long long rows, int C, float slope, int relu_in,
                                int need_dscale, int final_partials, hipStream_t s) {
  const int groups = C / V;
  const int nblocks = affine_bwd_blocks(rows, C), xcd = g_xpt_xcd_affinity && nblocks >= 8;
  const dim3 grid(xcd ? xpt_xcd_pad(nblocks) : nblocks, (groups + PW_MAX_GROUPS - 1) / PW_MAX_GROUPS);
  hipLaunchKernelGGL((affine_act_bwd_kernel<T, V>), grid, dim3(256), 0, s, (const T*)x, (const T*)y, (const T*)dy,
                     dy_pitch, a, (T*)dx, part, rows, C, affine_bwd_rows_per_block(rows), slope, relu_in, need_dscale,
                     final_partials, nblocks, xcd);
}

static void affine_bwd_launch(const void* x, const void* y, const void* dy, long long dy_pitch, const Affine& a,
                              void* dx, float* part, long long rows, int C, float slope, int relu_in, int need_dscale,
                              int final_partials, int dtype, hipStream_t s) {
  const int esz = dtype == 0 ? 4 : 2;
  int v = dtype == 0 ? 4 : 8;
  auto ok = [&](const void* p, long long pitch) {
    return p == nullptr || (((uintptr_t)p) % (size_t)(v * esz) == 0 && pitch % v == 0);
  };
  while (v > 1 && !(C % v == 0 && ok(x, C) && ok(y, C) && ok(dy, dy_pitch) && ok(dx, C))) v >>= 1;
#define XPT_AFF(T, V) \
  affine_bwd_launch_v<T, V>(x, y, dy, dy_pitch, a, dx, part, rows, C, slope, relu_in, need_dscale, final_partials, s)
  if (dtype == 0) {
    if (v == 4) XPT_AFF(float, 4);
    else if (v == 2) XPT_AFF(float, 2);
    else XPT_AFF(float, 1);
  } else {
    if (v == 8) XPT_AFF(xpt_half_t, 8);
    else if (v == 4) XPT_AFF(xpt_half_t, 4);
    else if (v == 2) XPT_AFF(xpt_half_t, 2);
    else XPT_AFF(xpt_half_t, 1);
  }
#undef XPT_AFF
}

static int affine_bwd_check(const void* x, const void* y, const void* dy, const float* gamma, const float* beta,
                            const float* mean, const float* var, long long rows, int C, float slope, int relu_in,
                            int dtype) {
  XPT_CHECK_PTR(dy); XPT_CHECK_PTR(beta);
  if (slope != 1.f) XPT_CHECK_PTR(y);
  if (rows <= 0 || C <= 0) return XPT_ERR_SHAPE;
  if (dtype != 0 && dtype != 1) return XPT_ERR_ARG;
  if (gamma && (!mean || !var)) return XPT_ERR_NULL;
  if ((gamma || relu_in) && !x) return XPT_ERR_NULL;
  return XPT_OK;
}

}

extern "C" {

int xpt_affine_act_fwd(const void* x, const float* gamma, const float* beta, const float* mean, const float* var,
                       float eps, const void* residual, void* y, long long rows, int C, float slope, int relu_in,
                       int dtype, void* stream) {
  XPT_CHECK_PTR(x); XPT_CHECK_PTR(beta); XPT_CHECK_PTR(y);
  if (residual && slope != 1.f) return XPT_ERR_ARG;
  if (gamma && (!mean || !var)) return XPT_ERR_NULL;
  if (rows <= 0 || C <= 0) return XPT_ERR_SHAPE;
  if (dtype != 0 && dtype != 1) return XPT_ERR_ARG;
  const long long n = rows * C;
  if (n >= (1LL << 31)) return XPT_ERR_SHAPE;
  const Affine a{gamma, beta, mean, var, eps};
  const XcdSweep sw = xpt_xcd_sweep(n, 4096);
  XPT_BEGIN_LAUNCH();
  if (dtype == 0)
    hipLaunchKernelGGL(affine_act_fwd_kernel<float>, dim3(sw.grid), dim3(256), 0, (hipStream_t)stream,
                       (const float*)x, a, (const float*)residual, (float*)y, n, C, slope, relu_in, sw);
  else
    hipLaunchKernelGGL(affine_act_fwd_kernel<xpt_half_t>, dim3(sw.grid), dim3(256), 0, (hipStream_t)stream,
                       (const xpt_half_t*)x, a, (const xpt_half_t*)residual, (xpt_half_t*)y, n, C, slope,
                       relu_in, sw);
  return xpt_launch_status();
}

size_t xpt_affine_act_bwd_workspace_floats(long long rows, int C) {
  if (rows <= 0 || C <= 0) return 0;
  return (size_t)affine_bwd_blocks(rows, C) * 2 * (size_t)C;
}

int xpt_affine_act_bwd(const void* x, const void* y, const void* dy, long long dy_pitch, const float* gamma,
                       const float* beta, const float* mean, const float* var, float eps, void* dx, float* dbeta,
                       float* dgamma,
                       float* workspace, size_t workspace_floats, long long rows, int C, float slope, int relu_in,
                       int dtype, void* stream) {
  XPT_CHECK_PTR(dbeta); XPT_CHECK_PTR(workspace);
  const int rc = affine_bwd_check(x, y, dy, gamma, beta, mean, var, rows, C, slope, relu_in, dtype);
  if (rc != XPT_OK) return rc;
  if ((gamma == nullptr) != (dgamma == nullptr)) return XPT_ERR_ARG;
  if (workspace_floats < xpt_affine_act_bwd_workspace_floats(rows, C)) return XPT_ERR_WORKSPACE;
  const Affine a{gamma, beta, mean, var, eps};
  hipStream_t s = (hipStream_t)stream;
  XPT_BEGIN_LAUNCH();
  if (dy_pitch < C) return XPT_ERR_SHAPE;
  affine_bwd_launch(x, y, dy, dy_pitch, a, dx, workspace, rows, C, slope, relu_in, dgamma != nullptr, 0, dtype, s);
  hipLaunchKernelGGL(affine_finish_kernel, dim3((C + 3) / 4), dim3(256), 0, s, workspace, a, dbeta, dgamma, C,
                     affine_bwd_blocks(rows, C));
  return xpt_launch_status();
}

int xpt_affine_act_bwd_blocks(long long rows, int C) {
  if (rows <= 0 || C <= 0) return 0;
  return affine_bwd_blocks(rows, C);
}

int xpt_affine_act_bwd_partials(const void* x, const void* y, const void* dy, long long dy_pitch, const float* gamma,
                                const float* beta, const float* mean, const float* var, float eps, void* dx,
                                float* partials,
                                size_t partial_floats, long long rows, int C, float slope, int relu_in, int dtype,
                                void* stream) {
  XPT_CHECK_PTR(partials);
  const int rc = affine_bwd_check(x, y, dy, gamma, beta, mean, var, rows, C, slope, relu_in, dtype);
  if (rc != XPT_OK) return rc;
  if (partial_floats < (size_t)affine_bwd_blocks(rows, C) * 2 * (size_t)C) return XPT_ERR_WORKSPACE;
  const Affine a{gamma, beta, mean, var, eps};
  XPT_BEGIN_LAUNCH();
  if (dy_pitch < C) return XPT_ERR_SHAPE;
  affine_bwd_launch(x, y, dy, dy_pitch, a, dx, partials, rows, C, slope, relu_in, gamma != nullptr, 1, dtype,
                    (hipStream_t)stream);
  return xpt_launch_status();
}

int xpt_depth_head_fwd(const float* x, float* depth, float* disp, long long n, void* stream) {
  XPT_CHECK_PTR(x); XPT_CHECK_PTR(depth); XPT_CHECK_PTR(disp);
  if (n <= 0) return XPT_ERR_SHAPE;
  XPT_BEGIN_LAUNCH();
  hipLaunchKernelGGL(depth_head_fwd_kernel, dim3(grid_for(n)), dim3(256), 0, (hipStream_t)stream, x, depth, disp, n);
  return xpt_launch_status();
}

int xpt_depth_head_bwd(const float* x, const float* g_depth, const float* g_disp, float* gx, long long n, void* stream) {
  XPT_CHECK_PTR(x); XPT_CHECK_PTR(gx);
  if (!g_depth && !g_disp) return XPT_ERR_NULL;
  if (n <= 0) return XPT_ERR_SHAPE;
  XPT_BEGIN_LAUNCH();
  hipLaunchKernelGGL(depth_head_bwd_kernel, dim3(grid_for(n)), dim3(256), 0, (hipStream_t)stream, x, g_depth, g_disp, gx, n);
  return xpt_launch_status();
}

int xpt_global_avgpool_fwd(const void* x, float* y, int B, int HW, int C, int dtype, void* stream) {
  XPT_CHECK_PTR(x); XPT_CHECK_PTR(y);
  if (B <= 0 || HW <= 0 || C <= 0) return XPT_ERR_SHAPE;
  if (dtype != 0 && dtype != 1) return XPT_ERR_ARG;
  const int total = B * C;
  XPT_BEGIN_LAUNCH();
  if (dtype == 0)
    hipLaunchKernelGGL(gap_fwd_kernel<float>, dim3((total + 255) / 256), dim3(256), 0, (hipStream_t)stream,
                       (const float*)x, y, total, HW, C);
  else
    hipLaunchKernelGGL(gap_fwd_kernel<xpt_half_t>, dim3((total + 255) / 256), dim3(256), 0, (hipStream_t)stream,
                       (const xpt_half_t*)x, y, total, HW, C);
  return xpt_launch_status();
}

int xpt_global_avgpool_bwd(const float* g, void* dx, int B, int HW, int C, int dtype, void* stream) {
  XPT_CHECK_PTR(g); XPT_CHECK_PTR(dx);
  if (B <= 0 || HW <= 0 || C <= 0) return XPT_ERR_SHAPE;
  if (dtype != 0 && dtype != 1) return XPT_ERR_ARG;
  const long long total = (long long)B * HW * C;
  if (total >= (1LL << 31)) return XPT_ERR_SHAPE;
  XPT_BEGIN_LAUNCH();
  if (dtype == 0)
    hipLaunchKernelGGL(gap_bwd_kernel<float>, dim3(grid_for(total)), dim3(256), 0, (hipStream_t)stream, g, (float*)dx,
                       total, HW, C);
  else
    hipLaunchKernelGGL(gap_bwd_kernel<xpt_half_t>, dim3(grid_for(total)), dim3(256), 0, (hipStream_t)stream, g,
                       (xpt_half_t*)dx, total, HW, C);
  return xpt_launch_status();
}

int xpt_upsample2x_fwd(const float* src, void* out, long long M, int h, int w, int dtype, void* stream) {
  XPT_CHECK_PTR(src); XPT_CHECK_PTR(out);
  if (M <= 0 || h <= 0 || w <= 0) return XPT_ERR_SHAPE;
  if (dtype != 0 && dtype != 1) return XPT_ERR_ARG;
  const long long total = M * 4 * h * w;
  if (total >= 0x7fffffffLL) return XPT_ERR_SHAPE;
  const XcdSweep sw = xpt_xcd_sweep(total, 4096);
  XPT_BEGIN_LAUNCH();
  if (dtype == 0)
    hipLaunchKernelGGL(upsample2x_fwd_kernel<float>, dim3(sw.grid), dim3(256), 0, (hipStream_t)stream, src,
                       (float*)out, total, h, w, sw);
  else
    hipLaunchKernelGGL(upsample2x_fwd_kernel<xpt_half_t>, dim3(sw.grid), dim3(256), 0, (hipStream_t)stream,
                       src, (xpt_half_t*)out, total, h, w, sw);
  return xpt_launch_status();
}

int xpt_upsample2x_bwd_add(const void* g, long long g_pitch, const float* addend, float* dsrc, long long M, int h, int w, int dtype,
                           void* stream) {
  XPT_CHECK_PTR(g); XPT_CHECK_PTR(dsrc);
  if (M <= 0 || h <= 0 || w <= 0 || g_pitch < 1) return XPT_ERR_SHAPE;
  if (dtype != 0 && dtype != 1) return XPT_ERR_ARG;
  const long long total = M * h * w;
  if (total >= 0x7fffffffLL) return XPT_ERR_SHAPE;
  const XcdSweep sw = xpt_xcd_sweep(total, 4096);
  XPT_BEGIN_LAUNCH();
  if (dtype == 0)
    hipLaunchKernelGGL(upsample2x_bwd_kernel<float>, dim3(sw.grid), dim3(256), 0, (hipStream_t)stream,
                       (const float*)g, g_pitch, addend, dsrc, total, h, w, sw);
  else
    hipLaunchKernelGGL(upsample2x_bwd_kernel<xpt_half_t>, dim3(sw.grid), dim3(256), 0, (hipStream_t)stream,
                       (const xpt_half_t*)g, g_pitch, addend, dsrc, total, h, w, sw);
  return xpt_launch_status();
}

int xpt_upsample2x_bwd(const void* g, long long g_pitch, float* dsrc, long long M, int h, int w, int dtype, void* stream) {
  return xpt_upsample2x_bwd_add(g, g_pitch, nullptr, dsrc, M, h, w, dtype, stream);
}

int xpt_depth_head_ms_fwd(int nscales, const float* const* x, float* const* depth, float* const* disp, const long long* n,
                          void* stream) {
  XPT_CHECK_PTR(x); XPT_CHECK_PTR(depth); XPT_CHECK_PTR(disp); XPT_CHECK_PTR(n);
  if (nscales < 1 || nscales > 4) return XPT_ERR_SHAPE;
  DepthHeadMs a = {};
  long long most = 0;
  for (int s = 0; s < nscales; ++s) {
    if (!x[s] || !depth[s] || !disp[s]) return XPT_ERR_NULL;
    if (n[s] <= 0) return XPT_ERR_SHAPE;
    a.x[s] = x[s]; a.depth[s] = depth[s]; a.disp[s] = disp[s]; a.n[s] = n[s];
    if (n[s] > most) most = n[s];
  }
  XPT_BEGIN_LAUNCH();
  hipLaunchKernelGGL(depth_head_ms_fwd_kernel, dim3(grid_for(most), nscales), dim3(256), 0, (hipStream_t)stream, a);
  return xpt_launch_status();
}

int xpt_depth_head_ms_bwd(int nscales, const float* const* x, const float* const* g_depth, const float* const* g_disp,
                          float* const* gx, const long long* n, void* stream) {
  XPT_CHECK_PTR(x); XPT_CHECK_PTR(g_depth); XPT_CHECK_PTR(g_disp); XPT_CHECK_PTR(gx); XPT_CHECK_PTR(n);
  if (nscales < 1 || nscales > 4) return XPT_ERR_SHAPE;
  DepthHeadMs a = {};
  long long most = 0;
  for (int s = 0; s < nscales; ++s) {
    if (!x[s] || !gx[s]) return XPT_ERR_NULL;
    if (n[s] <= 0) return XPT_ERR_SHAPE;
    a.x[s] = x[s]; a.depth[s] = gx[s]; a.g_depth[s] = g_depth[s]; a.g_disp[s] = g_disp[s]; a.n[s] = n[s];
    if (n[s] > most) most = n[s];
  }
  XPT_BEGIN_LAUNCH();
  hipLaunchKernelGGL(depth_head_ms_bwd_kernel, dim3(grid_for(most), nscales), dim3(256), 0, (hipStream_t)stream, a);
  return xpt_launch_status();
}

int xpt_avgpool3_same(const void* in, long long in_pitch, void* out, int B, int H, int W, int C, float scale, int adjoint,
                      int dtype, void* stream) {
  XPT_CHECK_PTR(in); XPT_CHECK_PTR(out);
  if (B <= 0 || H <= 0 || W <= 0 || C <= 0 || in_pitch < C) return XPT_ERR_SHAPE;
  if ((dtype != 0 && dtype != 1) || (adjoint != 0 && adjoint != 1)) return XPT_ERR_ARG;
  const int esz = dtype == 0 ? 4 : 2;
  int v = dtype == 0 ? 4 : 8;
  while (v > 1 && !(C % v == 0 && in_pitch % v == 0 && ((uintptr_t)in) % (size_t)(v * esz) == 0 &&
                    ((uintptr_t)out) % (size_t)(v * esz) == 0))
    v >>= 1;
  const long long total = (long long)B * H * W * (C / v);
  if (total >= (1LL << 31)) return XPT_ERR_SHAPE;
  const dim3 grid(grid_for(total));
  hipStream_t s = (hipStream_t)stream;
  XPT_BEGIN_LAUNCH();
#define XPT_POOL(T, V) \
  hipLaunchKernelGGL((avgpool3_kernel<T, V>), grid, dim3(256), 0, s, (const T*)in, in_pitch, (T*)out, B, H, W, C, scale, adjoint)
  if (dtype == 0) {
    if (v == 4) XPT_POOL(float, 4);
    else if (v == 2) XPT_POOL(float, 2);
    else XPT_POOL(float, 1);
  } else {
    if (v == 8) XPT_POOL(xpt_half_t, 8);
    else if (v == 4) XPT_POOL(xpt_half_t, 4);
    else if (v == 2) XPT_POOL(xpt_half_t, 2);
    else XPT_POOL(xpt_half_t, 1);
  }
#undef XPT_POOL
  return xpt_launch_status();
}

int xpt_sum_rows(const void* const* inputs, const long long* pitches, int n, void* out, long long rows, int C, int dtype,
                 void* stream) {
  XPT_CHECK_PTR(inputs); XPT_CHECK_PTR(pitches); XPT_CHECK_PTR(out);
  if (n < 2 || n > 8) return XPT_ERR_ARG;
  if (rows <= 0 || C <= 0) return XPT_ERR_SHAPE;
  if (dtype != 0 && dtype != 1) return XPT_ERR_ARG;
  SumInputs in;
  in.n = n;
  const int esz = dtype == 0 ? 4 : 2;
  int v = dtype == 0 ? 4 : 8;
  for (int i = 0; i < n; ++i) {
    if (inputs[i] == nullptr) return XPT_ERR_NULL;
    if (pitches[i] < C) return XPT_ERR_SHAPE;
    in.ptr[i] = inputs[i];
    in.pitch[i] = pitches[i];
  }
  auto ok = [&](const void* p, long long pitch) { return ((uintptr_t)p) % (size_t)(v * esz) == 0 && pitch % v == 0; };
  for (;;) {
    bool all = C % v == 0 && ok(out, C);
    for (int i = 0; i < n && all; ++i) all = ok(inputs[i], pitches[i]);
    if (all || v == 1) break;
    v >>= 1;
  }
  const long long total = rows * (C / v);
  if (total >= (1LL << 31)) return XPT_ERR_SHAPE;
  const XcdSweep sw = xpt_xcd_sweep(total, 4096);
  const dim3 grid(sw.grid);
  hipStream_t s = (hipStream_t)stream;
  XPT_BEGIN_LAUNCH();
#define XPT_SUM(T, V) hipLaunchKernelGGL((sum_rows_kernel<T, V>), grid, dim3(256), 0, s, in, (T*)out, rows, C, sw)
  if (dtype == 0) {
    if (v == 4) XPT_SUM(float, 4);
    else if (v == 2) XPT_SUM(float, 2);
    else XPT_SUM(float, 1);
  } else {
    if (v == 8) XPT_SUM(xpt_half_t, 8);
    else if (v == 4) XPT_SUM(xpt_half_t, 4);
    else if (v == 2) XPT_SUM(xpt_half_t, 2);
    else XPT_SUM(xpt_half_t, 1);
  }
#undef XPT_SUM
  return xpt_launch_status();
}

int xpt_multi_copy(const void* const* src, void* const* dst, const long long* bytes, int n, void* stream) {
  XPT_CHECK_PTR(src); XPT_CHECK_PTR(dst); XPT_CHECK_PTR(bytes);
  if (n < 1 || n > 8) return XPT_ERR_ARG;
  CopyJobs jobs{};
  jobs.n = n;
  long long vecs = 0;
  for (int i = 0; i < n; ++i) {
    if (src[i] == nullptr || dst[i] == nullptr) return XPT_ERR_NULL;
    if (bytes[i] <= 0) return XPT_ERR_SHAPE;
    jobs.src[i] = (const unsigned char*)src[i];
    jobs.dst[i] = (unsigned char*)dst[i];
    jobs.bytes[i] = bytes[i];
    jobs.first[i] = vecs;
    vecs += (bytes[i] + 15) / 16;
  }
  for (int i = n; i <= 8; ++i) jobs.first[i] = vecs;
  long long blocks = (vecs + 255) / 256;
  if (blocks > 4096) blocks = 4096;
  XPT_BEGIN_LAUNCH();
  hipLaunchKernelGGL(multi_copy_kernel, dim3((unsigned)blocks), dim3(256), 0, (hipStream_t)stream, jobs);
  return xpt_launch_status();
}

int xpt_concat_channels(const void* const* inputs, const long long* pitches, const int* channels, int n, void* out,
                        long long rows, int Ct, void* stream) {
  XPT_CHECK_PTR(inputs); XPT_CHECK_PTR(pitches); XPT_CHECK_PTR(channels); XPT_CHECK_PTR(out);
  if (n < 1 || n > 4) return XPT_ERR_ARG;
  if (rows <= 0 || Ct <= 0 || Ct % 8 != 0 || ((uintptr_t)out) % 16 != 0) return XPT_ERR_SHAPE;
  CatInputs in{};
  in.n = n;
  int c = 0;
  for (int i = 0; i < n; ++i) {
    if (inputs[i] == nullptr) return XPT_ERR_NULL;
    if (channels[i] <= 0 || pitches[i] < channels[i]) return XPT_ERR_SHAPE;
    in.ptr[i] = (const unsigned short*)inputs[i];
    in.pitch[i] = pitches[i];
    in.first[i] = c;
    c += channels[i];
  }
  for (int i = n; i <= 4; ++i) in.first[i] = c;
  if (c > Ct) return XPT_ERR_SHAPE;
  const long long total = rows * (Ct / 8);
  if (total >= (1LL << 31)) return XPT_ERR_SHAPE;
  XPT_BEGIN_LAUNCH();
  const XcdSweep sw = xpt_xcd_sweep(total, 4096);
  hipLaunchKernelGGL(concat_channels_kernel, dim3(sw.grid), dim3(256), 0, (hipStream_t)stream, in,
                     (unsigned short*)out, (unsigned)total, Ct / 8, sw);
  return xpt_launch_status();
}

}
```

### xpt_mde_2021_amd/hip/conv.py

```python
import contextlib
import ctypes
import math
import weakref

import torch

from . import lib as _lib
from . import ops as _ops


def _stream():
    return torch.cuda.current_stream().cuda_stream


def round_up(n, m):
    return (n + m - 1) // m * m


def same_pad(n, k, s):
    total = max((math.ceil(n / s) - 1) * s + k - n, 0)
    return total // 2, total - total // 2


class ConvWeightPacker:

    def __init__(self):
        self.entries = {}
        self.signature = None
        self.table = None
        self.retired = []
        self.nblocks = 0

    def get(self, weight, need_bwd=True):
        e = self.entries.get(id(weight))
        if e is not None and e["ref"]() is weight:
            if need_bwd and e["bwd"] is None:
                if torch.cuda.is_current_stream_capturing():
                    raise _lib.XptHipError("ConvWeightPacker: new operand layout requested during graph capture")
                e["bwd"] = torch.zeros((e["Cp"], e["T"], e["Np"]), dtype=_lib.half(), device=weight.device)
                self.signature = None
                self._pack_now()
            return e
        if torch.cuda.is_current_stream_capturing():
            raise _lib.XptHipError("ConvWeightPacker: a convolution weight was first used during graph capture "
                                   "(run one eager step first)")
        N, C, KH, KW = weight.shape
        Cp, Np, T = round_up(C, 8), round_up(N, 8), KH * KW
        e = {"ref": weakref.ref(weight), "N": N, "C": C, "KH": KH, "KW": KW, "T": T, "Cp": Cp, "Np": Np,
             "fwd": torch.zeros((N, T, Cp), dtype=_lib.half(), device=weight.device),
             "bwd": torch.zeros((Cp, T, Np), dtype=_lib.half(), device=weight.device) if need_bwd else None}
        self.entries[id(weight)] = e
        self.signature = None
        self._pack_now()
        return e

    def _live(self):
        dead = [k for k, e in self.entries.items() if e["ref"]() is None]
        for k in dead:
            del self.entries[k]
        if dead:
            self.signature = None
        return [(e["ref"](), e) for e in self.entries.values()]

    def _pack_now(self):
        if not torch.cuda.is_current_stream_capturing():
            self.pack()

    def pack(self):
        live = self._live()
        live = [(w, e) for w, e in live if w is not None and w.is_cuda]
        if not live:
            return
        lib = _lib.load()
        sig = tuple((w.data_ptr(), w.stride(), e["fwd"].data_ptr(), 0 if e["bwd"] is None else e["bwd"].data_ptr())
                    for w, e in live)
        if sig != self.signature:
            if torch.cuda.is_current_stream_capturing():
                raise _lib.XptHipError("ConvWeightPacker: the set of convolution weights changed during graph capture")
            assert lib.xpt_conv_pack_job_bytes() == ctypes.sizeof(_lib.ConvPackJob)
            jobs = (_lib.ConvPackJob * len(live))()
            first = 0
            for j, (w, e) in enumerate(live):
                if w.dtype != torch.float32:
                    raise _lib.XptHipError("ConvWeightPacker: master weights must be float32")
                sn, sc, sh, sw = w.stride()
                job = jobs[j]
                job.src, job.fwd, job.bwd = w.data_ptr(), e["fwd"].data_ptr(), (None if e["bwd"] is None else e["bwd"].data_ptr())
                job.sn, job.sc, job.sh, job.sw = sn, sc, sh, sw
                job.N, job.T, job.KW, job.C, job.Cp, job.Np = e["N"], e["T"], e["KW"], e["C"], e["Cp"], e["Np"]
                job.first_block = first
                first += e["T"] * ((max(e["N"], e["Np"]) + 63) // 64) * ((e["Cp"] + 63) // 64)
            if self.table is not None:
                self.retired.append(self.table)
            self.table = torch.frombuffer(bytearray(bytes(jobs)), dtype=torch.uint8).to(live[0][0].device)
            self.nblocks = first
            self.signature = sig
        _lib.check(lib.xpt_conv_pack_weights(self.table.data_ptr(), len(live), self.nblocks, _stream()),
                   "xpt_conv_pack_weights")


packer = ConvWeightPacker()


def _apply_env_tuning():
    import os
    spec = os.environ.get("XPT_WGRAD_TUNE")
    if spec:
        mib, blocks = (int(v) for v in spec.split(","))
        _lib.load().xpt_conv2d_bwd_weight_tune(mib, blocks)
    spec = os.environ.get("XPT_PW_WGRAD_TUNE")
    if spec:
        _lib.load().xpt_conv1x1_bwd_weight_tune(*[int(v) for v in spec.split(",")])
    if os.environ.get("XPT_XCD_AFFINITY"):
        _lib.load().xpt_set_xcd_affinity(int(os.environ["XPT_XCD_AFFINITY"]))
    for code in os.environ.get("XPT_DW_TUNE", "").split(","):
        if code:
            _lib.load().xpt_dwconv_tune(int(code))
    plan = os.environ.get("XPT_CONV_TUNE")
    if plan:
        for code in plan.split(","):
            _lib.load().xpt_conv2d_tune(int(code))
    spec = os.environ.get("XPT_SPLITK_TUNE")
    if spec:
        _lib.load().xpt_conv2d_splitk_tune(*[int(v) for v in spec.split(",")])
    spec = os.environ.get("XPT_STREAM_TUNE")
    if spec:
        _lib.load().xpt_conv2d_stream_tune(*[int(v) for v in spec.split(",")])
    spec = os.environ.get("XPT_PWCONV_TUNE")
    if spec:
        _lib.load().xpt_pwconv_tune(*[int(v) for v in spec.split(",")])
    spec = os.environ.get("XPT_HEAD_TUNE")
    if spec:
        _lib.load().xpt_headconv_tune(*[int(v) for v in spec.split(",")])
    cap = os.environ.get("XPT_PW_DEFER_CAP_MIB")
    if cap:
        _lib.load().xpt_conv1x1_bwd_weight_defer_cap(int(cap))


def nhwc_view(t, channels=None):
    if t.dtype != _lib.half() or not t.is_cuda:
        raise _lib.XptHipError("conv: expected a bfloat16 CUDA/HIP tensor (no CPU fallback)")
    B, C, H, W = t.shape
    sb, sc, sh, sw = t.stride()
    ok = sc == 1 and sh == W * sw and sb == H * sh and sw >= C and sw % 8 == 0 and t.data_ptr() % 16 == 0
    if not ok or B * H * W == 1:
        t = t.contiguous(memory_format=torch.channels_last)
        if t.stride(1) != 1:
            t = t.permute(0, 2, 3, 1).contiguous().permute(0, 3, 1, 2)
        sw = C
        if C % 8 != 0:
            raise _lib.XptHipError(f"conv: {C} channels are not a multiple of 8 (pad the tensor)")
    return t, sw


_tuned = False


class _Conv2dSame(torch.autograd.Function):

    @staticmethod
    def forward(ctx, x, weight, bias, stride, slope, upsample, valid):
        lib = _lib.load()
        global _tuned
        if not _tuned:
            _apply_env_tuning()
            _tuned = True
        x, xpitch = nhwc_view(x)
        B, Cx, PH, PW = x.shape
        need_dx = ctx.needs_input_grad[0]
        e = packer.get(weight, need_bwd=need_dx)
        N, C, KH, KW, Cp = e["N"], e["C"], e["KH"], e["KW"], e["Cp"]
        if Cx != Cp:
            raise _lib.XptHipError(f"conv: input has {Cx} channels, the packed weight expects {Cp} (= {C} padded to 8)")
        H, W = PH << upsample, PW << upsample
        if valid:
            pt = pl = 0
            OH, OW = (H - KH) // stride + 1, (W - KW) // stride + 1
        else:
            (pt, _), (pl, _) = same_pad(H, KH, stride), same_pad(W, KW, stride)
            OH, OW = -(-H // stride), -(-W // stride)
        y = torch.empty((B, N, OH, OW), dtype=_lib.half(), device=x.device, memory_format=torch.channels_last)
        b_ = None if bias is None else bias.detach()
        if b_ is not None and (b_.dtype != torch.float32 or not b_.is_contiguous()):
            raise _lib.XptHipError("conv: bias must be a contiguous float32 vector")
        wsf = 0 if valid else lib.xpt_conv2d_splitk_workspace_floats(B * OH * OW, N, Cp, KH * KW, stride)
        if wsf:
            ws = torch.empty(wsf, dtype=torch.float32, device=x.device)
            _lib.check(lib.xpt_conv2d_fwd_splitk(x.data_ptr(), e["fwd"].data_ptr(), None if b_ is None else b_.data_ptr(),
                                                 y.data_ptr(), B, PH, PW, Cp, xpitch, N, KH, KW, pt, pl, OH, OW, N,
                                                 int(upsample), float(slope), ws.data_ptr(), wsf, _stream()),
                       "xpt_conv2d_fwd_splitk")
        elif not valid and KH == 5 and lib.xpt_conv2d_stream_serves(B, OH, OW, N, Cp, KH, KW, stride, int(upsample)):
            _lib.check(lib.xpt_conv2d_fwd_stream_k5s2(x.data_ptr(), e["fwd"].data_ptr(), None if b_ is None else b_.data_ptr(),
                                                      y.data_ptr(), B, PH, PW, Cp, xpitch, N, pt, pl, OH, OW, N, float(slope),
                                                      _stream()), "xpt_conv2d_fwd_stream_k5s2")
        elif not valid and KH == 3 and lib.xpt_conv2d_stream_serves(B, OH, OW, N, Cp, KH, KW, stride, int(upsample)):
            _lib.check(lib.xpt_conv2d_fwd_stream(x.data_ptr(), e["fwd"].data_ptr(), None if b_ is None else b_.data_ptr(),
                                                 y.data_ptr(), B, PH, PW, Cp, xpitch, N, pt, pl, OH, OW, N, int(upsample),
                                                 float(slope), _stream()), "xpt_conv2d_fwd_stream")
        else:
            _lib.check(lib.xpt_conv2d_fwd(x.data_ptr(), e["fwd"].data_ptr(), None if b_ is None else b_.data_ptr(),
                                          y.data_ptr(), B, PH, PW, Cp, xpitch, N, KH, KW, stride, pt, pl, OH, OW, N,
                                          int(upsample), float(slope), _stream()), "xpt_conv2d_fwd")
        ctx.save_for_backward(x, y if slope != 1.0 else None, b_)
        ctx.geom = (B, PH, PW, Cp, C, xpitch, N, KH, KW, stride, pt, pl, OH, OW, int(upsample), float(slope))
        ctx.weight = weight
        ctx.sink_w = weight.flat_grad if (_ops.grad_sink.wants(weight) and N % 8 == 0) else None
        ctx.sink_b = bias.flat_grad if (bias is not None and _ops.grad_sink.wants(bias)) else None
        ctx.has_bias = bias is not None
        return y

    @staticmethod
    def backward(ctx, dy_in):
        lib = _lib.load()
        x, y, bias = ctx.saved_tensors
        B, PH, PW, Cp, C, xpitch, N, KH, KW, stride, pt, pl, OH, OW, ups, slope = ctx.geom
        weight = ctx.weight
        rows = B * OH * OW
        dy, dpitch = _ops._rows_with_pitch(dy_in.to(_lib.half()))
        dbias = None
        if ctx.has_bias or slope != 1.0:
            g = torch.empty((B, N, OH, OW), dtype=_lib.half(), device=dy.device, memory_format=torch.channels_last)
            if ctx.sink_b is not None:
                nblk = lib.xpt_affine_act_bwd_blocks(rows, N)
                ws = _ops.grad_sink.partials(ctx.sink_b, "affine", nblk * 2 * N)
                _lib.check(lib.xpt_affine_act_bwd_partials(None, None if y is None else y.data_ptr(), dy.data_ptr(), dpitch,
                                                           None, bias.data_ptr(), None, None, 0.0, g.data_ptr(),
                                                           ws.data_ptr(), ws.numel(), rows, N, slope, 0, 1, _stream()),
                           "xpt_affine_act_bwd_partials")
                _ops.grad_sink.add(ctx.sink_b, ws, 0, N, nblk, 2 * N)
            else:
                beta = bias if bias is not None else torch.zeros(N, dtype=torch.float32, device=dy.device)
                dbias = torch.empty(N, dtype=torch.float32, device=dy.device)
                nws = lib.xpt_affine_act_bwd_workspace_floats(rows, N)
                ws = torch.empty(nws, dtype=torch.float32, device=dy.device)
                _lib.check(lib.xpt_affine_act_bwd(None, None if y is None else y.data_ptr(), dy.data_ptr(), dpitch, None,
                                                  beta.data_ptr(), None, None, 0.0, g.data_ptr(), dbias.data_ptr(), None,
                                                  ws.data_ptr(), nws, rows, N, slope, 0, 1, _stream()), "xpt_affine_act_bwd")
                if not ctx.has_bias:
                    dbias = None
            gpitch = N
        else:
            g, gpitch = nhwc_view(dy_in.to(_lib.half()))
        if N % 8 != 0:
            raise _lib.XptHipError(f"conv backward: {N} output channels are not a multiple of 8")
        dx = dw = None
        if ctx.needs_input_grad[1]:
            if ctx.sink_w is not None and WGRAD_DEFER and getattr(weight, "defer_wgrad", False):
                _deferred.append((ctx, g, gpitch, x))
                side = None
            else:
                side = _wgrad_side_stream(g.device) if (ctx.sink_w is not None and WGRAD_SIDE_STREAM) else None
            if _deferred and _deferred[-1][0] is ctx:
                pass
            elif side is not None:
                side.wait_stream(torch.cuda.current_stream())
                g.record_stream(side)
                x.record_stream(side)
                _ops.grad_sink.join_streams.add(side)
            if not (_deferred and _deferred[-1][0] is ctx):
                with torch.cuda.stream(side) if side is not None else contextlib.nullcontext():
                    dw = _weight_grad(ctx, lib, g, gpitch, x)
        if ctx.needs_input_grad[0]:
            e = packer.get(weight, need_bwd=True)
            dx = torch.empty((B, Cp, PH, PW), dtype=_lib.half(), device=g.device, memory_format=torch.channels_last)
            wsf = lib.xpt_conv2d_splitk_workspace_floats(B * (PH << ups) * (PW << ups), Cp, e["Np"], KH * KW, stride)
            if wsf:
                ws = torch.empty(wsf, dtype=torch.float32, device=g.device)
                _lib.check(lib.xpt_conv2d_bwd_data_splitk(g.data_ptr(), e["bwd"].data_ptr(), dx.data_ptr(), B, OH, OW, e["Np"],
                                                          gpitch, Cp, KH, KW, pt, pl, PH, PW, Cp, ups, ws.data_ptr(), wsf,
                                                          _stream()), "xpt_conv2d_bwd_data_splitk")
            elif KH == 3 and lib.xpt_conv2d_stream_serves(B, PH << ups, PW << ups, Cp, e["Np"], KH, KW, stride, ups):
                _lib.check(lib.xpt_conv2d_bwd_data_stream(g.data_ptr(), e["bwd"].data_ptr(), dx.data_ptr(), B, OH, OW, e["Np"],
                                                          gpitch, Cp, pt, pl, PH, PW, Cp, ups, _stream()),
                           "xpt_conv2d_bwd_data_stream")
            else:
                _lib.check(lib.xpt_conv2d_bwd_data(g.data_ptr(), e["bwd"].data_ptr(), dx.data_ptr(), B, OH, OW, e["Np"], gpitch,
                                                   Cp, KH, KW, stride, pt, pl, PH, PW, Cp, ups, _stream()), "xpt_conv2d_bwd_data")
        if _deferred and getattr(weight, "flush_wgrads", False):
            _flush_deferred(True)
        return dx, dw, dbias, None, None, None, None


WGRAD_DEFER = __import__("os").environ.get("XPT_WGRAD_DEFER", "0") == "1"
_deferred = []


def _flush_deferred(to_side):
    global _deferred
    queue, _deferred = _deferred, []
    if not queue:
        return
    lib = _lib.load()
    side = _wgrad_side_stream(queue[0][1].device) if to_side else None
    if side is not None:
        side.wait_stream(torch.cuda.current_stream())
        _ops.grad_sink.join_streams.add(side)
    with torch.cuda.stream(side) if side is not None else contextlib.nullcontext():
        for ctx, g, gpitch, x in queue:
            if side is not None:
                g.record_stream(side)
                x.record_stream(side)
            _weight_grad(ctx, lib, g, gpitch, x)


WGRAD_SIDE_STREAM = __import__("os").environ.get("XPT_WGRAD_SIDE_STREAM", "0") == "1"
_SIDE = {}


def _wgrad_side_stream(device):
    if device not in _SIDE:
        _SIDE[device] = torch.cuda.Stream(device=device)
    return _SIDE[device]


def _weight_grad(ctx, lib, g, gpitch, x):
    B, PH, PW, Cp, C, xpitch, N, KH, KW, stride, pt, pl, OH, OW, ups, slope = ctx.geom
    nsplit = lib.xpt_conv2d_bwd_weight_splits(B, Cp, N, KH, KW, stride, OH, OW)
    if nsplit < 1:
        raise _lib.XptHipError(f"xpt_conv2d_bwd_weight_splits failed: {nsplit}")
    n = N * KH * KW * C
    if ctx.sink_w is not None:
        ws = _ops.grad_sink.partials(ctx.sink_w, "convw", nsplit * n)
    else:
        ws = torch.empty(nsplit * n, dtype=torch.float32, device=g.device)
    _lib.check(lib.xpt_conv2d_bwd_weight_partials(g.data_ptr(), x.data_ptr(), ws.data_ptr(), ws.numel(), B, PH, PW, Cp, C,
                                                  xpitch, N, gpitch, KH, KW, stride, pt, pl, OH, OW, ups, _stream()),
               "xpt_conv2d_bwd_weight_partials")
    if ctx.sink_w is not None:
        _ops.grad_sink.add(ctx.sink_w, ws, 0, n, nsplit, n)
        return None
    if torch.cuda.is_current_stream_capturing():
        raise _lib.XptHipError("conv weight gradient without a flat-gradient destination inside a graph capture")
    return ws[:nsplit * n].view(nsplit, N, KH, KW, C).sum(0).permute(0, 3, 1, 2)


def conv2d_same(x, weight, bias, stride=1, slope=1.0, upsample=False, valid=False):
    return _Conv2dSame.apply(x, weight, bias, int(stride), float(slope), bool(upsample), bool(valid))


def usable(x, conv, slope):
    if not x.is_cuda or slope is None or conv.groups != 1 or conv.dilation != (1, 1):
        return False
    dtype = torch.get_autocast_dtype("cuda") if torch.is_autocast_enabled() else x.dtype
    k = conv.kernel_size
    return dtype == _lib.half() and k[0] == k[1] and k[0] in (1, 3, 5) and conv.out_channels % 8 == 0 \
        and conv.weight.dtype == torch.float32


def stem_input_usable(image):
    if not (torch.is_tensor(image) and image.is_cuda and image.dtype == torch.float32 and image.dim() == 4
            and image.shape[1] == 3 and torch.is_autocast_enabled() and torch.get_autocast_dtype("cuda") == _lib.half()):
        return False
    sb, sc, sh, sw = image.stride()
    return sc == 1 and sw == 3 and sh == 3 * image.shape[3] and sb >= 3 * image.shape[2] * image.shape[3]


def stem_input(image):
    lib = _lib.load()
    B, _, H, W = image.shape
    out = torch.empty((B, 8, H + 2, W + 2), dtype=_lib.half(), device=image.device, memory_format=torch.channels_last)
    _lib.check(lib.xpt_stem_input(image.data_ptr(), image.stride(0), out.data_ptr(), B, H, W, _stream()), "xpt_stem_input")
    return out


def restack_bf16(image5d, channels_padded):
    lib = _lib.load()
    if not image5d.is_cuda or image5d.dtype != torch.float32:
        raise _lib.XptHipError("restack_bf16: expected a float32 CUDA/HIP tensor")
    image5d = image5d.contiguous()
    B, S, H, W, C = image5d.shape
    if C != 3:
        raise _lib.XptHipError("restack_bf16: expected 3 channels per frame")
    out = torch.empty((B, H, W, channels_padded), dtype=_lib.half(), device=image5d.device)
    _lib.check(lib.xpt_restack_bf16(image5d.data_ptr(), out.data_ptr(), B, S, H, W, channels_padded, _stream()),
               "xpt_restack_bf16")
    return out.permute(0, 3, 1, 2)


class _HeadConv(torch.autograd.Function):

    @staticmethod
    def forward(ctx, x, weight, bias):
        lib = _lib.load()
        x, xpitch = nhwc_view(x)
        B, C, H, W = x.shape
        w = weight.detach()
        if w.dtype != torch.float32 or tuple(w.shape) != (1, C, 3, 3):
            raise _lib.XptHipError(f"head_conv: weight must be float32 [1, {C}, 3, 3], got {tuple(w.shape)} {w.dtype}")
        if not (w.stride(1) == 1 and w.stride(3) == C and w.stride(2) == 3 * C):
            w = w.permute(0, 2, 3, 1).contiguous().permute(0, 3, 1, 2)
        b_ = None if bias is None else bias.detach()
        pre = torch.empty((B, 1, H, W), dtype=torch.float32, device=x.device)
        _lib.check(lib.xpt_headconv_fwd(x.data_ptr(), xpitch, w.data_ptr(), None if b_ is None else b_.data_ptr(),
                                        pre.data_ptr(), B, H, W, C, _stream()), "xpt_headconv_fwd")
        ctx.save_for_backward(x, w)
        ctx.geom = (B, C, H, W, xpitch)
        ctx.sink = None
        if _ops.grad_sink.wants(weight) and weight.flat_grad.numel() == 9 * C and (bias is None or _ops.grad_sink.wants(bias)):
            ctx.sink = (weight.flat_grad, None if bias is None else bias.flat_grad)
        ctx.has_bias = bias is not None
        return pre

    @staticmethod
    def backward(ctx, g):
        lib = _lib.load()
        x, w = ctx.saved_tensors
        B, C, H, W, xpitch = ctx.geom
        g = g.contiguous().float()
        dx = torch.empty((B, C, H, W), dtype=_lib.half(), device=g.device, memory_format=torch.channels_last)
        nblk = lib.xpt_headconv_bwd_blocks(B, H, W, C)
        row = 9 * C + 1
        if ctx.sink is not None:
            ws = _ops.grad_sink.partials(ctx.sink[0], "head", nblk * row)
        else:
            ws = torch.empty(nblk * row, dtype=torch.float32, device=g.device)
        _lib.check(lib.xpt_headconv_bwd(x.data_ptr(), xpitch, w.data_ptr(), g.data_ptr(), dx.data_ptr(), ws.data_ptr(),
                                        ws.numel(), B, H, W, C, _stream()), "xpt_headconv_bwd")
        if ctx.sink is not None:
            _ops.grad_sink.add(ctx.sink[0], ws, 0, 9 * C, nblk, row)
            if ctx.sink[1] is not None:
                _ops.grad_sink.add(ctx.sink[1], ws, 9 * C, 1, nblk, row)
            return dx, None, None
        tot = ws[:nblk * row].view(nblk, row).sum(0)
        dw = tot[:9 * C].view(1, 3, 3, C).permute(0, 3, 1, 2)
        return dx, dw, (tot[9 * C:].clone() if ctx.has_bias else None)


class _HeadConvSplit(_HeadConv):

    @staticmethod
    def forward(ctx, x, weight, bias):
        pre = _HeadConv.forward(ctx, x, weight, bias)
        ctx.set_materialize_grads(False)
        return pre, x.view_as(x)

    @staticmethod
    def backward(ctx, g, g_x):
        lib = _lib.load()
        x, w = ctx.saved_tensors
        B, C, H, W, xpitch = ctx.geom
        if g is None:
            return g_x, None, None
        g = g.contiguous().float()
        add, apitch = (None, 0)
        if g_x is not None:
            add, apitch = nhwc_view(g_x.to(_lib.half()))
        dx = torch.empty((B, C, H, W), dtype=_lib.half(), device=g.device, memory_format=torch.channels_last)
        nblk = lib.xpt_headconv_bwd_blocks(B, H, W, C)
        row = 9 * C + 1
        if ctx.sink is not None:
            ws = _ops.grad_sink.partials(ctx.sink[0], "head", nblk * row)
        else:
            ws = torch.empty(nblk * row, dtype=torch.float32, device=g.device)
        _lib.check(lib.xpt_headconv_bwd_add(x.data_ptr(), xpitch, w.data_ptr(), g.data_ptr(), None if add is None else add.data_ptr(),
                                            apitch, dx.data_ptr(), ws.data_ptr(), ws.numel(), B, H, W, C, _stream()),
                   "xpt_headconv_bwd_add")
        if ctx.sink is not None:
            _ops.grad_sink.add(ctx.sink[0], ws, 0, 9 * C, nblk, row)
            if ctx.sink[1] is not None:
                _ops.grad_sink.add(ctx.sink[1], ws, 9 * C, 1, nblk, row)
            return dx, None, None
        tot = ws[:nblk * row].view(nblk, row).sum(0)
        dw = tot[:9 * C].view(1, 3, 3, C).permute(0, 3, 1, 2)
        return dx, dw, (tot[9 * C:].clone() if ctx.has_bias else None)


def head_conv_split(x, weight, bias):
    return _HeadConvSplit.apply(x, weight, bias)


def head_conv(x, weight, bias):
    return _HeadConv.apply(x, weight, bias)


def head_usable(x, conv):
    return x.is_cuda and x.dtype == _lib.half() and conv.in_channels in (16, 32, 64, 128) and conv.out_channels == 1 \
        and conv.kernel_size == (3, 3) and conv.weight.dtype == torch.float32 and conv.dilation == (1, 1) and conv.stride == (1, 1)


_ops.grad_sink.pre_flush.append(lambda: _flush_deferred(False))
```

### xpt_mde_2021_amd/hip/lib.py

```python
import ctypes
import os

_HERE = os.path.dirname(os.path.abspath(__file__))
LIB_PATH = os.environ.get("XPT_HIP_LIB") or os.path.join(os.path.dirname(_HERE), "libxpt_hip.so")
LIB_PATH_F16 = os.environ.get("XPT_HIP_LIB_F16") or os.path.join(os.path.dirname(_HERE), "libxpt_hip_f16.so")

_half_format = os.environ.get("XPT_HALF", "bf16")


def set_half_format(fmt):
    global _half_format
    if fmt not in ("bf16", "fp16"):
        raise XptHipError(f"unknown 16-bit format {fmt!r} (bf16 | fp16)")
    if _lib is not None and fmt != _half_format:
        raise XptHipError(f"the {_half_format} build of the library is already loaded in this process: {fmt} needs its own process "
                          f"(XPT_HALF={fmt} in the environment, or set_half_format() before the first op)")
    _half_format = fmt


def half_format():
    return _half_format


_half_dtype = None


def half():
    global _half_dtype
    if _half_dtype is None or _half_dtype[0] != _half_format:
        import torch
        _half_dtype = (_half_format, torch.float16 if _half_format == "fp16" else torch.bfloat16)
    return _half_dtype[1]

XPT_PHOTO_L1, XPT_PHOTO_L2, XPT_PHOTO_SSIM = 0, 1, 2
PHOTO_METHODS = {"L1": XPT_PHOTO_L1, "L2": XPT_PHOTO_L2, "SSIM": XPT_PHOTO_SSIM}

_ERRORS = {-1: "XPT_ERR_NULL (required pointer is NULL)", -2: "XPT_ERR_SHAPE (bad dimension)",
           -3: "XPT_ERR_ARG (bad enum/flag)", -4: "XPT_ERR_WORKSPACE (workspace too small)",
           -5: "XPT_ERR_LAUNCH (hipGetLastError != hipSuccess)"}

_p = ctypes.c_void_p
_i = ctypes.c_int
_f = ctypes.c_float
_z = ctypes.c_size_t

SIGNATURES = {
    "xpt_abi_version": (_i, []),
    "xpt_build_arch": (ctypes.c_char_p, []),
    "xpt_pose_rvec2matr_fwd": (_i, [_p, _p, _i, _p]),
    "xpt_pose_rvec2matr_bwd": (_i, [_p, _p, _p, _i, _p]),
    "xpt_resize_down_fwd": (_i, [_p, _p, _i, _i, _i, _i, _i, _p]),
    "xpt_image_pyramids": (_i, [_p, _i, _i, _i, _i, _i, _p, _p, _p, _p, _p]),
    "xpt_warp_fwd": (_i, [_p, _p, _p, _p, _p, _i, _i, _i, _i, _f, _p]),
    "xpt_warp_bwd_workspace_floats": (_z, [_i, _i, _i, _i]),
    "xpt_warp_bwd": (_i, [_p, _p, _p, _p, _p, _p, _p, _p, _z, _i, _i, _i, _i, _f, _p]),
    "xpt_bilinear_fwd": (_i, [_p, _p, _p, _p, _i, _i, _i, _i, _i, _i, _p]),
    "xpt_bilinear_bwd": (_i, [_p, _p, _p, _p, _p, _i, _i, _i, _i, _i, _i, _p]),
    "xpt_photo_workspace_floats": (_z, [_i, _i, _i, _i]),
    "xpt_photo_fwd": (_i, [_i, _p, _p, _p, _p, _p, _z, _i, _i, _i, _i, _p]),
    "xpt_photo_bwd": (_i, [_i, _p, _p, _p, _p, _p, _p, _z, _i, _i, _i, _i, _p]),
    "xpt_photo_fused_tune": (_i, [_i, _i, _i]),
    "xpt_photo_fused_variant": (_i, [_i]),
    "xpt_photo_fused_workspace_floats": (_z, [_i, _i, _i, _i]),
    "xpt_photo_fused_fwd": (_i, [_p, _p, _p, _p, _p, _p, _p, _p, _p, _z, _i, _i, _i, _i, _f, _p]),
    "xpt_photo_fused_bwd": (_i, [_p, _p, _p, _p, _p, _p, _p, _p, _p, _p, _z, _i, _i, _i, _i, _f, _p]),
    "xpt_smooth_workspace_floats": (_z, [_i, _i, _i]),
    "xpt_smooth_fwd": (_i, [_p, _p, _p, _p, _z, _i, _i, _i, _f, _i, _p]),
    "xpt_smooth_bwd": (_i, [_p, _p, _p, _p, _i, _i, _i, _f, _i, _p]),
    "xpt_merge_total_fwd": (_i, [_i, _p, _p, _p, _p, _p, _i, _i, _p]),
    "xpt_merge_total_bwd": (_i, [_i, _p, _p, _p, _i, _p]),
    "xpt_smooth_ms_fwd": (_i, [_i, _p, _p, _p, _p, _z, _i, _p, _p, _f, _i, _p]),
    "xpt_smooth_ms_bwd": (_i, [_i, _p, _p, _p, _p, _i, _p, _p, _f, _i, _p]),
    "xpt_adam_step": (_i, [_p, _p, _p, _p, ctypes.c_longlong, _p, _f, _f, _f, _f, _f, _i, _p, _p]),
    "xpt_sgd_step": (_i, [_p, _p, ctypes.c_longlong, _f, _f, _i, _p, _p]),
    "xpt_grad_nonfinite": (_i, [_p, ctypes.c_longlong, _p, _p]),
    "xpt_loss_scale_update": (_i, [_p, _i, _p]),
    "xpt_adam_step_dyn": (_i, [_p, _p, _p, _p, ctypes.c_longlong, _p, _f, _f, _f, _f, _f, _i, _p, _p, _p]),
    "xpt_sgd_step_dyn": (_i, [_p, _p, ctypes.c_longlong, _f, _f, _i, _p, _p, _p]),
    "xpt_dwconv_fwd": (_i, [_p, _p, _p] + [_i] * 12 + [_p]),
    "xpt_dwconv_bwd_data": (_i, [_p, _p, _p, _p] + [_i] * 12 + [_p]),
    "xpt_dwconv_tune": (_i, [_i]),
    "xpt_dwconv_bwd_weight_workspace_floats": (_z, [_i] * 5),
    "xpt_dwconv_bwd_weight": (_i, [_p, _p, _p, _p, _z] + [_i] * 12 + [_p]),
    "xpt_conv1x1_bwd_weight_workspace_floats": (_z, [ctypes.c_longlong, _i, _i]),
    "xpt_conv1x1_bwd_weight_tune": (_i, [_i, _i, _i, _i]),
    "xpt_conv1x1_bwd_weight_counters": (_i, [ctypes.c_longlong, _i, _i]),
    "xpt_conv1x1_bwd_weight": (_i, [_p, _p, _p, _p, _z, _p, _i, ctypes.c_longlong, _i, _i, ctypes.c_longlong,
                                    ctypes.c_longlong, _p]),
    "xpt_reduce_job_bytes": (_i, []),
    "xpt_reduce_partials": (_i, [_p, _p, _i, _p]),
    "xpt_half_format": (_i, []),
    "xpt_affine_act_bwd_blocks": (_i, [ctypes.c_longlong, _i]),
    "xpt_affine_act_bwd_partials": (_i, [_p, _p, _p, ctypes.c_longlong, _p, _p, _p, _p, _f, _p, _p, _z, ctypes.c_longlong,
                                         _i, _f, _i, _i, _p]),
    "xpt_dwconv_bwd_weight_chunks": (_i, [_i] * 6),
    "xpt_set_xcd_affinity": (_i, [_i]),
    "xpt_dwconv_bwd_weight_partials": (_i, [_p, _p, _p, _z] + [_i] * 12 + [_p]),
    "xpt_dwconv_bwd_both": (_i, [_p, _p, _p, _p, _p, _z] + [_i] * 12 + [_p]),
    "xpt_dwconv_multi_fwd": (_i, [_p, _p, _p, _p, _p, _p] + [_i] * 10 + [_p]),
    "xpt_dwconv_multi_bwd": (_i, [_p, _p, _i, _p, _p, _p, _p, _p, _p, _p] + [_i] * 10 + [_p]),
    "xpt_conv1x1_bwd_weight_defer_cap": (_i, [_i]),
    "xpt_conv1x1_bwd_weight_splits": (_i, [ctypes.c_longlong, _i, _i]),
    "xpt_conv1x1_bn_bwd_partials": (_i, [_p, _p, _p, _p, _p, _p, _f, _p, _p, _z, _p, _z, ctypes.c_longlong, _i, _i,
                                         ctypes.c_longlong, ctypes.c_longlong, _p]),
    "xpt_conv1x1_bn_bwd_partials_sum": (_i, [_p, _p, _p, _p, _p, _p, _p, _p, _f, _p, _p, _z, _p, _z, ctypes.c_longlong, _i, _i,
                                             ctypes.c_longlong, ctypes.c_longlong, ctypes.c_longlong, ctypes.c_longlong, _p]),
    "xpt_conv1x1_bwd_fused": (_i, [_p, _p, _p, _p, _p, _z, ctypes.c_longlong, _i, _i, ctypes.c_longlong, ctypes.c_longlong, _p]),
    "xpt_conv1x1_bn_bwd_fused": (_i, [_p, _p, _p, _p, _p, _p, _p, _p, _p, _f, _p, _p, _z, _p, _z, ctypes.c_longlong, _i, _i,
                                      ctypes.c_longlong, ctypes.c_longlong, ctypes.c_longlong, ctypes.c_longlong, _p]),
    "xpt_conv1x1_bn_multi_bwd_fused": (_i, [_i, _p, _p, _p, _p, _p, _p, _p, _p, _f, _p, _p, _p, _z, _z, ctypes.c_longlong,
                                            _i, _i, ctypes.c_longlong, _p]),
    "xpt_conv1x1_bn_multi_bwd_fused_fan": (_i, [_i, _p, _p, _p, _p, _p, _p, _p, _p, _p, _p, _p, _p, _f, _p, _p, _p, _z, _z,
                                                ctypes.c_longlong, _i, _i, ctypes.c_longlong, _p]),
    "xpt_conv1x1_bn_multi_bwd_partials": (_i, [_i, _p, _p, _p, _p, _p, _p, _p, _f, _p, _p, _p, _z, _z, ctypes.c_longlong, _i, _i,
                                               ctypes.c_longlong, _p]),
    "xpt_conv1x1_bwd_weight_partials": (_i, [_p, _p, _p, _z, ctypes.c_longlong, _i, _i, ctypes.c_longlong,
                                             ctypes.c_longlong, _p]),
    "xpt_pwconv_bn_fwd": (_i, [_p, _p, _p, _p, _p, _p, _f, _p, _p, _p, ctypes.c_longlong, _i, _i, ctypes.c_longlong, _p]),
    "xpt_multi_copy": (_i, [_p, _p, _p, _i, _p]),
    "xpt_concat_channels": (_i, [_p, _p, _p, _i, _p, ctypes.c_longlong, _i, _p]),
    "xpt_avgpool3_same": (_i, [_p, ctypes.c_longlong, _p, _i, _i, _i, _i, _f, _i, _i, _p]),
    "xpt_pwconv_bn_multi_fwd": (_i, [_i, _p, _p, _p, _p, _p, _p, _f, _p, _p, _p, ctypes.c_longlong, _i, _i, ctypes.c_longlong, _p]),
    "xpt_pwconv_bn_multi_fwd_sib": (_i, [_i, _p, _p, _p, _p, _p, _p, _f, _p, _p, _p, _p, _p, _p, _p, _p, _p, _p,
                                         ctypes.c_longlong, _i, _i, ctypes.c_longlong, ctypes.c_longlong, _p]),
    "xpt_corr_cost_channels": (_i, [_i, _i]),
    "xpt_corr_cost_fwd": (_i, [_p, _p, _p, _i, _i, _i, _i, _i, _i, _i, _p]),
    "xpt_corr_cost_bwd": (_i, [_p, _p, _p, _p, _p, _i, _i, _i, _i, _i, _i, _i, _p]),
    "xpt_headconv_tune": (_i, [_i, _i]),
    "xpt_pwconv_tune": (_i, [_i, _i]),
    "xpt_depth_head_fwd": (_i, [_p, _p, _p, ctypes.c_longlong, _p]),
    "xpt_depth_head_bwd": (_i, [_p, _p, _p, _p, ctypes.c_longlong, _p]),
    "xpt_global_avgpool_fwd": (_i, [_p, _p, _i, _i, _i, _i, _p]),
    "xpt_global_avgpool_bwd": (_i, [_p, _p, _i, _i, _i, _i, _p]),
    "xpt_upsample2x_fwd": (_i, [_p, _p, ctypes.c_longlong, _i, _i, _i, _p]),
    "xpt_upsample2x_bwd": (_i, [_p, ctypes.c_longlong, _p, ctypes.c_longlong, _i, _i, _i, _p]),
    "xpt_upsample2x_bwd_add": (_i, [_p, ctypes.c_longlong, _p, _p, ctypes.c_longlong, _i, _i, _i, _p]),
    "xpt_depth_head_ms_fwd": (_i, [_i, _p, _p, _p, _p, _p]),
    "xpt_depth_head_ms_bwd": (_i, [_i, _p, _p, _p, _p, _p, _p]),
    "xpt_sum_rows": (_i, [_p, _p, _i, _p, ctypes.c_longlong, _i, _i, _p]),
    "xpt_photo_fused_ms_fwd": (_i, [_i, _p, _p, _p, _p, _p, _p, _p, _z, _i, _i, _p, _p, _p, _p]),
    "xpt_photo_fused_ms_bwd": (_i, [_i, _p, _p, _p, _p, _p, _p, _p, _p, _p, _p, _z, _i, _i, _p, _p, _p, _p]),
    "xpt_graph_node_census": (_i, [_p, _p]),
    "xpt_sepconv_bn_multi_fwd": (_i, [_i] + [_p] * 23 + [_f, _i, _i, _i, _i, _i, _p]),
    "xpt_photo_march_tune": (_i, [_i, _i, _i]),
    "xpt_photo_march_plan": (_i, [_i, _i, _i, _i, _i]),
    "xpt_photo_march_ms_fwd": (_i, [_i, _p, _p, _p, _p, _p, _p, _p, _z, _i, _i, _p, _p, _p, _p]),
    "xpt_photo_march_ms_bwd": (_i, [_i, _p, _p, _p, _p, _p, _p, _p, _p, _p, _p, _z, _i, _i, _p, _p, _p, _p]),
    "xpt_photo_march_ms_fwdbwd": (_i, [_i, _p, _p, _p, _p, _p, _p, _p, _p, _p, _p, _p, _z, _i, _i, _p, _p, _p, _p]),
    "xpt_augment_pin": (_i, [_p]),
    "xpt_augment": (_i, [_p, _p, _p, _p, _p, _p, _i, _p, _p, _i, _p, _p, _p, _p, _i, _p, _p, _p, _p, _i, _p, _p, _i, _i,
                         _f, _f, _f, _f, _p]),
    "xpt_stem_input": (_i, [_p, ctypes.c_longlong, _p, _i, _i, _i, _p]),
    "xpt_pose_metric": (_i, [_p, _p, _p, _i, _i, _p]),
    "xpt_depth_metric": (_i, [_p, _p, _p, _i, _i, _i, _i, _i, _i, _i, _f, _f, _p]),
    "xpt_adjust_gather": (_i, [_p, ctypes.c_longlong, _p, _i, _i, _i, _i, _i, _p]),
    "xpt_adjust_scatter": (_i, [_p, ctypes.c_longlong, _p, ctypes.c_longlong, _p, _i, _i, _i, _i, _i, _p]),
    "xpt_pool_pair_fwd": (_i, [_p, ctypes.c_longlong, _p, _p, _p, _i, _i, _i, _i, _i, _i, _i, _i, _i, _p]),
    "xpt_pool_pair_bwd": (_i, [_p, ctypes.c_longlong, _p, ctypes.c_longlong, _p, _p, _i, _i, _i, _i, _i, _i, _i, _i, _i, _p]),
    "xpt_pool_pair_bwd2": (_i, [_p, ctypes.c_longlong, _p, ctypes.c_longlong, _p, ctypes.c_longlong, _p, _p, _i, _i, _i, _i, _i, _i,
                                _i, _i, _i, _p]),
    "xpt_cell_tail_fwd": (_i, [_i, _p, _p, _p, _p, _p, _p, ctypes.c_longlong, _i, _i, _i, _i, _i, _p]),
    "xpt_cell_tail_bwd": (_i, [_i, _p, _p, _p, ctypes.c_longlong, _p, _i, _i, _p, _p, _p, _p, _p, _i, _i, _i, _i, _i, _p]),
    "xpt_crc32c": (ctypes.c_uint32, [_p, _z]),
    "xpt_tfrecord_index": (ctypes.c_longlong, [_p, _z, _i, _p, _p, _p, ctypes.c_longlong]),
    "xpt_tfrecord_decode": (_i, [_p, _z, ctypes.c_uint32, _i, _i, _p, _p, _p]),
    "xpt_conv_pack_job_bytes": (_i, []),
    "xpt_conv_pack_weights": (_i, [_p, _i, ctypes.c_longlong, _p]),
    "xpt_conv2d_tune": (_i, [_i]),
    "xpt_conv2d_fwd": (_i, [_p, _p, _p, _p, _i, _i, _i, _i, ctypes.c_longlong, _i, _i, _i, _i, _i, _i, _i, _i,
                            ctypes.c_longlong, _i, _f, _p]),
    "xpt_conv2d_bwd_data": (_i, [_p, _p, _p, _i, _i, _i, _i, ctypes.c_longlong, _i, _i, _i, _i, _i, _i, _i, _i,
                                 ctypes.c_longlong, _i, _p]),
    "xpt_conv2d_splitk_tune": (_i, [_i, _i, _i, _i]),
    "xpt_conv2d_splitk_workspace_floats": (_z, [ctypes.c_longlong, _i, _i, _i, _i]),
    "xpt_conv2d_fwd_splitk": (_i, [_p, _p, _p, _p, _i, _i, _i, _i, ctypes.c_longlong, _i, _i, _i, _i, _i, _i, _i,
                                   ctypes.c_longlong, _i, _f, _p, _z, _p]),
    "xpt_conv2d_bwd_data_splitk": (_i, [_p, _p, _p, _i, _i, _i, _i, ctypes.c_longlong, _i, _i, _i, _i, _i, _i, _i,
                                        ctypes.c_longlong, _i, _p, _z, _p]),
    "xpt_conv2d_stream_tune": (_i, [_i, _i, _i, _i]),
    "xpt_conv2d_stream_serves": (_i, [_i] * 9),
    "xpt_conv2d_fwd_stream": (_i, [_p, _p, _p, _p, _i, _i, _i, _i, ctypes.c_longlong, _i, _i, _i, _i, _i, ctypes.c_longlong,
                                   _i, _f, _p]),
    "xpt_conv2d_fwd_stream_k5s2": (_i, [_p, _p, _p, _p, _i, _i, _i, _i, ctypes.c_longlong, _i, _i, _i, _i, _i, ctypes.c_longlong,
                                        _f, _p]),
    "xpt_conv2d_bwd_data_stream": (_i, [_p, _p, _p, _i, _i, _i, _i, ctypes.c_longlong, _i, _i, _i, _i, _i, ctypes.c_longlong,
                                        _i, _p]),
    "xpt_conv2d_bwd_weight_tune": (_i, [_i, _i]),
    "xpt_conv2d_bwd_weight_splits": (_i, [_i] * 8),
    "xpt_conv2d_bwd_weight_partials": (_i, [_p, _p, _p, _z, _i, _i, _i, _i, _i, ctypes.c_longlong, _i, ctypes.c_longlong,
                                            _i, _i, _i, _i, _i, _i, _i, _i, _p]),
    "xpt_headconv_bwd_blocks": (_i, [_i, _i, _i, _i]),
    "xpt_headconv_fwd": (_i, [_p, ctypes.c_longlong, _p, _p, _p, _i, _i, _i, _i, _p]),
    "xpt_headconv_bwd": (_i, [_p, ctypes.c_longlong, _p, _p, _p, _p, _z, _i, _i, _i, _i, _p]),
    "xpt_headconv_bwd_add": (_i, [_p, ctypes.c_longlong, _p, _p, _p, ctypes.c_longlong, _p, _p, _z, _i, _i, _i, _i, _p]),
    "xpt_restack_bf16": (_i, [_p, _p, _i, _i, _i, _i, _i, _p]),
    "xpt_affine_act_fwd": (_i, [_p, _p, _p, _p, _p, _f, _p, _p, ctypes.c_longlong, _i, _f, _i, _i, _p]),
    "xpt_affine_act_bwd_workspace_floats": (_z, [ctypes.c_longlong, _i]),
    "xpt_affine_act_bwd": (_i, [_p, _p, _p, ctypes.c_longlong, _p, _p, _p, _p, _f, _p, _p, _p, _p, _z, ctypes.c_longlong,
                                _i, _f, _i, _i, _p]),
    "xpt_dwconv_bn_relu6_fwd": (_i, [_p, _p, _p, _p, _p, _p, _f, _p] + [_i] * 10 + [_p]),
    "xpt_dwconv_bn_relu6_tune": (_i, [_i]),
    "xpt_dwconv_bn_relu6_fwd_outputs": (_i, [_i] * 4),
    "xpt_dwconv_bn_relu6_bwd_chunks": (_i, [_i] * 4),
    "xpt_dwconv_bn_relu6_bwd": (_i, [_p, _p, _p, ctypes.c_longlong, _p, _p, _p, _p, _f, _p, _p, _z] + [_i] * 10 + [_p]),
}



class ConvPackJob(ctypes.Structure):
    _fields_ = [("src", ctypes.c_void_p), ("fwd", ctypes.c_void_p), ("bwd", ctypes.c_void_p),
                ("sn", ctypes.c_longlong), ("sc", ctypes.c_longlong), ("sh", ctypes.c_longlong), ("sw", ctypes.c_longlong),
                ("N", ctypes.c_int), ("T", ctypes.c_int), ("KW", ctypes.c_int), ("C", ctypes.c_int), ("Cp", ctypes.c_int),
                ("Np", ctypes.c_int), ("first_block", ctypes.c_longlong)]


class ReduceJob(ctypes.Structure):
    _fields_ = [("dst", ctypes.c_void_p), ("n", ctypes.c_longlong), ("nseg", ctypes.c_int),
                ("split_waves", ctypes.c_int), ("src", ctypes.c_void_p * 4), ("stride", ctypes.c_longlong * 4),
                ("nsplit", ctypes.c_int * 4)]


_lib = None


class XptHipError(RuntimeError):
    pass


def load():
    global _lib
    if _lib is not None:
        return _lib
    path = LIB_PATH_F16 if _half_format == "fp16" else LIB_PATH
    if not os.path.isfile(path):
        raise XptHipError(f"HIP extension not built: {path} is missing. Run `python -c 'import __graft_entry__ as g; "
                          f"g.build()'` (hipcc --offload-arch=gfx950). There is no CPU fallback for these ops.")
    import torch
    lib = ctypes.CDLL(path)
    for name, (restype, argtypes) in SIGNATURES.items():
        try:
            fn = getattr(lib, name)
        except AttributeError as e:
            raise XptHipError(f"{path} does not export {name}; rebuild the extension") from e
        fn.restype = restype
        fn.argtypes = argtypes
    if lib.xpt_half_format() != (1 if _half_format == "fp16" else 0):
        raise XptHipError(f"{path} was not built for {_half_format} activations; rebuild the extension (csrc/build.py)")
    variant = os.environ.get("XPT_FUSED_FWD_PIPE")
    if variant is not None:
        lib.xpt_photo_fused_variant(int(variant))
    _lib = lib
    return lib


def check(code, what):
    if code != 0:
        raise XptHipError(f"{what} failed: {_ERRORS.get(code, code)}")
```

Measured before the change: 1959 images/sec.

## Fold activation backward and bias reduction into conv weight-gradient kernels

Adds an ACT variant of both weight-gradient kernels that applies the leaky-ReLU backward to dy on load, writes the activated gradient out for the data-gradient pass, and accumulates per-channel bias partials. The conv backward uses this fused path when the output-channel block count is small and the split count matches, skipping the separate affine/activation backward kernel and its extra read of dy. In exchange, blocks with c0==0 do extra global stores and a bias reduction through LDS, the y tensor is loaded in every channel block, and the wgrad is no longer deferred or put on a side stream for these layers.

Result: no change. 1973 images/sec, median of 2 (+0.7%).

```diff
diff --git a/include/xpt_hip.h b/include/xpt_hip.h
--- a/include/xpt_hip.h
+++ b/include/xpt_hip.h
@@ -194,6 +194,13 @@
 int xpt_conv2d_bwd_weight_partials(const void* g, const void* x, float* partials, size_t partial_floats, int B, int PH,
                                    int PW, int C, int Cr, long long xpitch, int N, long long gpitch, int KH, int KW,
                                    int stride, int pad_t, int pad_l, int OH, int OW, int upsample, void* stream);
+int xpt_conv2d_bwd_weight_act_blocks(int B, int PH, int PW, int C, int N, int KH, int KW, int stride, int pad_t, int pad_l,
+                                     int OH, int OW, int upsample);
+int xpt_conv2d_bwd_weight_act_partials(const void* dy, long long dy_pitch, const void* y, float slope, const void* x,
+                                       void* g_out, float* partials, size_t partial_floats, float* bias_partials,
+                                       size_t bias_floats, int B, int PH, int PW, int C, int Cr, long long xpitch, int N,
+                                       int KH, int KW, int stride, int pad_t, int pad_l, int OH, int OW, int upsample,
+                                       void* stream);
 int xpt_restack_bf16(const float* image5d, void* out, int B, int S, int H, int W, int Cp, void* stream);
 
 int xpt_headconv_tune(int passes, int max_blocks);
diff --git a/xpt_mde_2021_amd/csrc/xpt_common.h b/xpt_mde_2021_amd/csrc/xpt_common.h
--- a/xpt_mde_2021_amd/csrc/xpt_common.h
+++ b/xpt_mde_2021_amd/csrc/xpt_common.h
@@ -65,6 +65,24 @@
 #else
   return __float2bfloat16(f);
 #endif
+}
+__device__ __forceinline__ float xpt_act_bwd(float dy, float y, float slope) { return y > 0.f ? dy : dy * slope; }
+typedef unsigned int xpt_u32x4 __attribute__((ext_vector_type(4)));
+__device__ __forceinline__ xpt_u32x4 xpt_act_bwd_chunk(xpt_u32x4 dy, xpt_u32x4 y, float slope, bool has_y, float (&gf)[8]) {
+  xpt_u32x4 out;
+#pragma unroll
+  for (int k = 0; k < 4; ++k) {
+    float lo = xpt_h2f_lo(dy[k]), hi = xpt_h2f_hi(dy[k]);
+    if (has_y) {
+      lo = xpt_act_bwd(lo, xpt_h2f_lo(y[k]), slope);
+      hi = xpt_act_bwd(hi, xpt_h2f_hi(y[k]), slope);
+    }
+    gf[2 * k] = lo;
+    gf[2 * k + 1] = hi;
+    const xpt_half_t rl = xpt_float2half(lo), rh = xpt_float2half(hi);
+    out[k] = (unsigned)__builtin_bit_cast(unsigned short, rl) | ((unsigned)__builtin_bit_cast(unsigned short, rh) << 16);
+  }
+  return out;
 }
 #endif
 
diff --git a/xpt_mde_2021_amd/csrc/xpt_conv_wgrad.hip b/xpt_mde_2021_amd/csrc/xpt_conv_wgrad.hip
--- a/xpt_mde_2021_amd/csrc/xpt_conv_wgrad.hip
+++ b/xpt_mde_2021_amd/csrc/xpt_conv_wgrad.hip
@@ -20,6 +20,11 @@
   int R, CB, nseg, nrb, units, nsplit;
   int WN, WC, WT;
   int dbg;
+  const unsigned short* y;
+  unsigned short* gout;
+  float* bpart;
+  long long ybytes;
+  float slope;
 };
 
 __device__ inline bf16x8 tr_pair(const char* lds, unsigned off0, unsigned off1) {
@@ -67,9 +72,10 @@
   }
 }
 
-template <int MAXCH>
+template <int MAXCH, bool ACT>
 __device__ __forceinline__ void wgrad_fetch(const WgradArgs& a, int u, int gi, const WgradChunks<MAXCH>& w,
-                                            const __amdgpu_buffer_rsrc_t& rg, const __amdgpu_buffer_rsrc_t& rx, u32x4 (&stage)[MAXCH]) {
+                                            const __amdgpu_buffer_rsrc_t& rg, const __amdgpu_buffer_rsrc_t& rx,
+                                            const __amdgpu_buffer_rsrc_t& ry, u32x4 (&stage)[MAXCH], u32x4 (&sy)[ACT ? MAXCH : 1]) {
   unsigned seg, rb;
   const unsigned q1 = xpt_divmod((unsigned)u, (unsigned)a.nseg, seg);
   const unsigned b = xpt_divmod(q1, (unsigned)a.nrb, rb);
@@ -84,6 +90,12 @@
       const bool ok = r < a.OH && c < a.OW;
       const unsigned off = ok ? (gimg + (unsigned)(r * a.OW + c)) * gp2 + w.chb[i] : WG_OOB;
       stage[i] = __builtin_amdgcn_raw_buffer_load_b128(rg, off, 0, 0);
+      if constexpr (ACT) {
+        if (a.y) {
+          const unsigned yoff = ok ? (gimg + (unsigned)(r * a.OW + c)) * (unsigned)(a.N * 2) + w.chb[i] : WG_OOB;
+          sy[i] = __builtin_amdgcn_raw_buffer_load_b128(ry, yoff, 0, 0);
+        }
+      }
     } else {
       const int r = th0 + w.row[i], c = tw0 + w.col[i];
       const bool ok = r >= 0 && c >= 0 && r < a.Hlim && c < a.Wlim;
@@ -93,7 +105,7 @@
   }
 }
 
-template <int TAPS>
+template <int TAPS, bool ACT>
 __global__ __launch_bounds__(256) void conv_wgrad_kernel(WgradArgs a) {
   extern __shared__ __attribute__((aligned(16))) char smem[];
   const int tid = threadIdx.x, lane = tid & 63, wave = tid >> 6;
@@ -134,12 +146,39 @@
   constexpr int MAXCH = WGRAD_MAXCH;
   const __amdgpu_buffer_rsrc_t rg = __builtin_amdgcn_make_buffer_rsrc((void*)a.g, 0, (int)a.gbytes, 0x00020000);
   const __amdgpu_buffer_rsrc_t rx = __builtin_amdgcn_make_buffer_rsrc((void*)a.x, 0, (int)a.xbytes, 0x00020000);
-  u32x4 stage[MAXCH];
+  const __amdgpu_buffer_rsrc_t ry = __builtin_amdgcn_make_buffer_rsrc((void*)a.y, 0, ACT ? (int)a.ybytes : 0, 0x00020000);
+  u32x4 stage[MAXCH], sy[ACT ? MAXCH : 1] = {};
   WgradChunks<MAXCH> chunks;
   wgrad_chunks<MAXCH>(a, tid, n0, c0, TNB, TCB, Wt, gi, gchunks, xchunks, chunks);
+  const bool writer = ACT && c0 == 0;
+  float bsum[8];
+#pragma unroll
+  for (int j = 0; j < 8; ++j) bsum[j] = 0.f;
   int u = blockIdx.y;
-  if (u < a.units) wgrad_fetch<MAXCH>(a, u, gi, chunks, rg, rx, stage);
+  if (u < a.units) wgrad_fetch<MAXCH, ACT>(a, u, gi, chunks, rg, rx, ry, stage, sy);
   for (; u < a.units; u += a.nsplit) {
+    if constexpr (ACT) {
+      unsigned seg, rb;
+      const unsigned q1 = xpt_divmod((unsigned)u, (unsigned)a.nseg, seg);
+      const unsigned b = xpt_divmod(q1, (unsigned)a.nrb, rb);
+      const int oh0 = (int)rb * a.R, ow0 = (int)seg * a.CB;
+#pragma unroll
+      for (int i = 0; i < MAXCH; ++i) {
+        if (i < gi) {
+          float gf[8];
+          stage[i] = xpt_act_bwd_chunk(stage[i], sy[i], a.slope, a.y != nullptr, gf);
+          if (writer) {
+            const int r = oh0 + chunks.row[i], c = ow0 + chunks.col[i];
+            if (r < a.OH && c < a.OW && chunks.chb[i] != WG_OOB) {
+              const size_t pix = (size_t)b * (size_t)(a.OH * a.OW) + (size_t)(r * a.OW + c);
+              *(u32x4*)((char*)a.gout + pix * (size_t)(a.N * 2) + chunks.chb[i]) = stage[i];
+            }
+#pragma unroll
+            for (int j = 0; j < 8; ++j) bsum[j] += gf[j];
+          }
+        }
+      }
+    }
     __syncthreads();
 #pragma unroll
     for (int i = 0; i < MAXCH; ++i) {
@@ -148,7 +187,7 @@
     }
     __syncthreads();
     if (u + a.nsplit < a.units && !(a.dbg & 2))
-      wgrad_fetch<MAXCH>(a, u + a.nsplit, gi, chunks, rg, rx, stage);
+      wgrad_fetch<MAXCH, ACT>(a, u + a.nsplit, gi, chunks, rg, rx, ry, stage, sy);
     if (active && !(a.dbg & 1)) {
       for (int rr = 0; rr < a.R; ++rr) {
         for (int c16 = 0; c16 < a.CB; c16 += 16) {
@@ -167,6 +206,24 @@
     }
   }
 
+  if constexpr (ACT) {
+    if (writer) {
+      __syncthreads();
+      float* red = (float*)smem;
+#pragma unroll
+      for (int j = 0; j < 8; ++j) red[tid * 8 + j] = bsum[j];
+      __syncthreads();
+      const int G = TNB >> 3;
+      if (tid < TNB && n0 + tid < a.N) {
+        const int gc8 = tid >> 3, j = tid & 7;
+        float s0 = 0.f;
+        for (int k = 0; k < 256 / G; ++k) s0 += red[(k * G + gc8) * 8 + j];
+        float* row = a.bpart + (size_t)blockIdx.y * 2 * a.N;
+        row[n0 + tid] = s0;
+        row[a.N + n0 + tid] = 0.f;
+      }
+    }
+  }
   if (!active || (a.dbg & 4)) return;
   const int c = c0 + wc * 32 + (lane & 31);
   float* dst = a.part + (long long)blockIdx.y * a.N * T * a.Cr;
@@ -190,9 +247,15 @@
   int pad_t, pad_l, taps;
   int tiles_x, tiles_y, ntiles, nsplit, ct, nb;
   int xcd;
+  int perm;
+  const unsigned short* y;
+  unsigned short* gout;
+  float* bpart;
+  long long ybytes;
+  float slope;
 };
 
-template <int K, int S, bool UPS>
+template <int K, int S, bool UPS, bool ACT>
 __global__ __launch_bounds__(256) void conv_wgrad_fast_kernel(WfArgs a) {
   constexpr int HR = UPS ? 6 : 7 * S + K, WR = UPS ? 10 : 15 * S + K, HPIX = HR * WR;
   constexpr int T = K * K, TPW = (T + 3) / 4;
@@ -217,9 +280,12 @@
   const __amdgpu_buffer_rsrc_t rg = __builtin_amdgcn_make_buffer_rsrc((void*)a.g, 0, (int)a.gbytes, 0x00020000);
   const __amdgpu_buffer_rsrc_t rx = __builtin_amdgcn_make_buffer_rsrc((void*)a.x, 0, (int)a.xbytes, 0x00020000);
   const unsigned gp2 = (unsigned)(a.gpitch * 2), xp2 = (unsigned)(a.xpitch * 2);
+  const __amdgpu_buffer_rsrc_t ry = __builtin_amdgcn_make_buffer_rsrc((void*)a.y, 0, ACT ? (int)a.ybytes : 0, 0x00020000);
+  const unsigned yp2 = (unsigned)(a.N * 2);
+  const bool has_y = ACT && a.y != nullptr, writer = ACT && cblk == 0;
 
   int grow[NG], gcol[NG];
-  unsigned gcb[NG], gconst[NG];
+  unsigned gcb[NG], gconst[NG], yconst[ACT ? NG : 1];
 #pragma unroll
   for (int i = 0; i < NG; ++i) {
     const int v = tid + 256 * i, pix = v >> 2, cv = v & 3;
@@ -227,6 +293,7 @@
     gcol[i] = pix & 15;
     gcb[i] = n0 + cv * 8 < a.N ? (unsigned)(n0 + cv * 8) * 2u : WG_OOB;
     gconst[i] = (unsigned)(grow[i] * a.OW + gcol[i]) * gp2 + gcb[i];
+    if constexpr (ACT) yconst[i] = (unsigned)(grow[i] * a.OW + gcol[i]) * yp2 + gcb[i];
   }
   int xq[NX], xrem[NX], xlds[NX];
   unsigned xcb[NX], xconst[NX];
@@ -268,14 +335,17 @@
 
   auto tile_of = [&](int t, int& b, int& oh0, int& ow0) {
     unsigned u = (unsigned)t;
-    if (a.xcd) u = (u & 7u) * ((unsigned)a.ntiles >> 3) + (u >> 3);
+    if (a.perm) u = (u & 7u) * ((unsigned)a.ntiles >> 3) + (u >> 3);
     unsigned txi, tyi;
     const unsigned q1 = xpt_divmod(u, (unsigned)a.tiles_x, txi);
     b = __builtin_amdgcn_readfirstlane((int)xpt_divmod(q1, (unsigned)a.tiles_y, tyi));
     oh0 = __builtin_amdgcn_readfirstlane((int)tyi * 8);
     ow0 = __builtin_amdgcn_readfirstlane((int)txi * 16);
   };
-  u32x4 sg[NG], sx[NX];
+  u32x4 sg[NG], sx[NX], sy[ACT ? NG : 1] = {};
+  float bsum[8];
+#pragma unroll
+  for (int j = 0; j < 8; ++j) bsum[j] = 0.f;
   auto fetch = [&](int t) {
     int b, oh0, ow0;
     tile_of(t, b, oh0, ow0);
@@ -286,12 +356,26 @@
       const unsigned soff = (unsigned)((b * a.OH + oh0) * a.OW + ow0) * gp2;
 #pragma unroll
       for (int i = 0; i < NG; ++i) sg[i] = __builtin_amdgcn_raw_buffer_load_b128(rg, gconst[i], soff, 0);
+      if constexpr (ACT) {
+        if (has_y) {
+          const unsigned syoff = (unsigned)((b * a.OH + oh0) * a.OW + ow0) * yp2;
+#pragma unroll
+          for (int i = 0; i < NG; ++i) sy[i] = __builtin_amdgcn_raw_buffer_load_b128(ry, yconst[i], syoff, 0);
+        }
+      }
     } else {
 #pragma unroll
       for (int i = 0; i < NG; ++i) {
         const int r = oh0 + grow[i], c = ow0 + gcol[i];
-        const unsigned off = (r < a.OH && c < a.OW) ? (unsigned)((b * a.OH + r) * a.OW + c) * gp2 + gcb[i] : WG_OOB;
+        const bool ok = r < a.OH && c < a.OW;
+        const unsigned off = ok ? (unsigned)((b * a.OH + r) * a.OW + c) * gp2 + gcb[i] : WG_OOB;
         sg[i] = __builtin_amdgcn_raw_buffer_load_b128(rg, off, 0, 0);
+        if constexpr (ACT) {
+          if (has_y) {
+            const unsigned yoff = ok ? (unsigned)((b * a.OH + r) * a.OW + c) * yp2 + gcb[i] : WG_OOB;
+            sy[i] = __builtin_amdgcn_raw_buffer_load_b128(ry, yoff, 0, 0);
+          }
+        }
       }
     }
     if (x_in) {
@@ -312,6 +396,24 @@
   int t = split;
   if (t < a.ntiles) fetch(t);
   for (; t < a.ntiles; t += a.nsplit) {
+    if constexpr (ACT) {
+      int b, oh0, ow0;
+      tile_of(t, b, oh0, ow0);
+#pragma unroll
+      for (int i = 0; i < NG; ++i) {
+        float gf[8];
+        sg[i] = xpt_act_bwd_chunk(sg[i], sy[i], a.slope, has_y, gf);
+        if (writer) {
+          const int r = oh0 + grow[i], c = ow0 + gcol[i];
+          if (r < a.OH && c < a.OW && gcb[i] != WG_OOB) {
+            const size_t pix = (size_t)((b * a.OH + r) * a.OW + c);
+            *(u32x4*)((char*)a.gout + pix * (size_t)yp2 + gcb[i]) = sg[i];
+          }
+#pragma unroll
+          for (int j = 0; j < 8; ++j) bsum[j] += gf[j];
+        }
+      }
+    }
     __syncthreads();
 #pragma unroll
     for (int i = 0; i < NG; ++i) *(u32x4*)(gs + (tid + 256 * i) * 16) = sg[i];
@@ -335,6 +437,23 @@
     }
   }
 
+  if constexpr (ACT) {
+    if (writer) {
+      __syncthreads();
+      float* red = (float*)smem;
+#pragma unroll
+      for (int j = 0; j < 8; ++j) red[tid * 8 + j] = bsum[j];
+      __syncthreads();
+      if (tid < 32 && n0 + tid < a.N) {
+        const int cv = tid >> 3, j = tid & 7;
+        float s0 = 0.f;
+        for (int k = 0; k < 64; ++k) s0 += red[(4 * k + cv) * 8 + j];
+        float* row = a.bpart + (size_t)split * 2 * a.N;
+        row[n0 + tid] = s0;
+        row[a.N + n0 + tid] = 0.f;
+      }
+    }
+  }
   const int c = c0 + (lane & 31);
   float* dst = a.part + (long long)split * a.N * T * a.Cr;
 #pragma unroll
@@ -466,10 +585,26 @@
   return p.nsplit;
 }
 
-extern "C" int xpt_conv2d_bwd_weight_partials(const void* g, const void* x, float* partials, size_t partial_floats, int B,
-                                              int PH, int PW, int C, int Cr, long long xpitch, int N, long long gpitch,
-                                              int KH, int KW, int stride, int pad_t, int pad_l, int OH, int OW,
-                                              int upsample, void* stream) {
+namespace {
+
+struct ActFold {
+  const void* y;
+  void* gout;
+  float* bpart;
+  size_t bfloats;
+  float slope;
+};
+
+bool fast_serves(int B, int PH, int PW, int C, int N, int KH, int KW, int stride, int pad_t, int pad_l, int OH, int OW,
+                 int upsample, WfArgs& f) {
+  return fast_plan(B, C, N, KH, KW, stride, OH, OW, upsample, f) &&
+         (upsample ? ((long long)PH * 2 == OH && (long long)PW * 2 == OW && pad_t == 1 && pad_l == 1)
+                   : ((long long)(OH - 1) * stride - pad_t < PH && (long long)(OW - 1) * stride - pad_l < PW));
+}
+
+int wgrad_launch(const void* g, const void* x, float* partials, size_t partial_floats, int B, int PH, int PW, int C, int Cr,
+                 long long xpitch, int N, long long gpitch, int KH, int KW, int stride, int pad_t, int pad_l, int OH, int OW,
+                 int upsample, const ActFold* act, void* stream) {
   XPT_CHECK_PTR(g); XPT_CHECK_PTR(x); XPT_CHECK_PTR(partials);
   if (B <= 0 || PH <= 0 || PW <= 0 || C <= 0 || Cr <= 0 || Cr > C || N <= 0 || KH <= 0 || KW <= 0 || OH <= 0 || OW <= 0)
     return XPT_ERR_SHAPE;
@@ -478,11 +613,16 @@
     return XPT_ERR_ARG;
   {
     WfArgs f{};
-    if (fast_plan(B, C, N, KH, KW, stride, OH, OW, upsample, f) &&
-        (upsample ? ((long long)PH * 2 == OH && (long long)PW * 2 == OW && pad_t == 1 && pad_l == 1)
-                  : ((long long)(OH - 1) * stride - pad_t < PH && (long long)(OW - 1) * stride - pad_l < PW))) {
+    if (fast_serves(B, PH, PW, C, N, KH, KW, stride, pad_t, pad_l, OH, OW, upsample, f)) {
       f.nsplit = fast_nsplit(f, N, C);
       if (partial_floats < (size_t)f.nsplit * N * KH * KW * Cr) return XPT_ERR_WORKSPACE;
+      if (act) {
+        if (f.nsplit != xpt_conv2d_bwd_weight_splits(B, C, N, KH, KW, stride, OH, OW)) return XPT_ERR_ARG;
+        if (act->bfloats < (size_t)f.nsplit * 2 * N) return XPT_ERR_WORKSPACE;
+        f.y = (const unsigned short*)act->y; f.gout = (unsigned short*)act->gout; f.bpart = act->bpart;
+        f.ybytes = (long long)B * OH * OW * N * 2; f.slope = act->slope;
+        if (f.ybytes >= (1LL << 30)) return XPT_ERR_SHAPE;
+      }
       f.g = (const unsigned short*)g; f.x = (const unsigned short*)x; f.part = partials;
       f.gpitch = gpitch; f.xpitch = xpitch;
       f.gbytes = ((long long)B * OH * OW - 1) * gpitch * 2 + (long long)N * 2;
@@ -490,13 +630,20 @@
       if (f.gbytes >= (1LL << 30) || f.xbytes >= (1LL << 30)) return XPT_ERR_SHAPE;
       f.B = B; f.PH = PH; f.PW = PW; f.OH = OH; f.OW = OW; f.C = C; f.Cr = Cr; f.N = N; f.pad_t = pad_t; f.pad_l = pad_l;
       f.xcd = (g_xpt_xcd_affinity != 0 && f.ntiles % 8 == 0 && f.nsplit % 8 == 0) ? 1 : 0;
+      f.perm = act ? ((f.ntiles % 8 == 0 && f.nsplit % 8 == 0) ? 1 : 0) : f.xcd;
       const dim3 grid(f.ct * f.nb * f.nsplit);
       hipStream_t st = (hipStream_t)stream;
       XPT_BEGIN_LAUNCH();
-      if (upsample) hipLaunchKernelGGL((conv_wgrad_fast_kernel<3, 1, true>), grid, dim3(256), 0, st, f);
-      else if (KH == 3 && stride == 1) hipLaunchKernelGGL((conv_wgrad_fast_kernel<3, 1, false>), grid, dim3(256), 0, st, f);
-      else if (KH == 3) hipLaunchKernelGGL((conv_wgrad_fast_kernel<3, 2, false>), grid, dim3(256), 0, st, f);
-      else hipLaunchKernelGGL((conv_wgrad_fast_kernel<5, 2, false>), grid, dim3(256), 0, st, f);
+#define XPT_WF_LAUNCH(ACT)                                                                                              \
+  do {                                                                                                                 \
+    if (upsample) hipLaunchKernelGGL((conv_wgrad_fast_kernel<3, 1, true, ACT>), grid, dim3(256), 0, st, f);            \
+    else if (KH == 3 && stride == 1) hipLaunchKernelGGL((conv_wgrad_fast_kernel<3, 1, false, ACT>), grid, dim3(256), 0, st, f); \
+    else if (KH == 3) hipLaunchKernelGGL((conv_wgrad_fast_kernel<3, 2, false, ACT>), grid, dim3(256), 0, st, f);       \
+    else hipLaunchKernelGGL((conv_wgrad_fast_kernel<5, 2, false, ACT>), grid, dim3(256), 0, st, f);                    \
+  } while (0)
+      if (act) XPT_WF_LAUNCH(true);
+      else XPT_WF_LAUNCH(false);
+#undef XPT_WF_LAUNCH
       return xpt_launch_status();
     }
   }
@@ -515,13 +662,24 @@
   a.R = p.R; a.CB = p.CB; a.nseg = p.nseg; a.nrb = p.nrb; a.units = p.units; a.nsplit = p.nsplit;
   a.WN = p.WN; a.WC = p.WC; a.WT = p.WT;
   a.dbg = g_wgrad_dbg;
+  size_t lds = p.lds;
+  if (act) {
+    if (p.nsplit != xpt_conv2d_bwd_weight_splits(B, C, N, KH, KW, stride, OH, OW)) return XPT_ERR_ARG;
+    if (act->bfloats < (size_t)p.nsplit * 2 * N) return XPT_ERR_WORKSPACE;
+    a.y = (const unsigned short*)act->y; a.gout = (unsigned short*)act->gout; a.bpart = act->bpart;
+    a.ybytes = (long long)B * OH * OW * N * 2; a.slope = act->slope;
+    if (a.ybytes >= (1LL << 30)) return XPT_ERR_SHAPE;
+    a.dbg = 0;
+    if (lds < 8192) lds = 8192;
+  }
   const int TNB = 32 * p.WN, TCB = 32 * p.WC;
   const dim3 grid(((N + TNB - 1) / TNB) * ((C + TCB - 1) / TCB), p.nsplit);
   hipStream_t s = (hipStream_t)stream;
   XPT_BEGIN_LAUNCH();
 #define XPT_WGRAD_CASE(TP)                                                                                         \
   case TP: {                                                                                                       \
-    hipLaunchKernelGGL(conv_wgrad_kernel<TP>, grid, dim3(256), p.lds, s, a);                                       \
+    if (act) hipLaunchKernelGGL((conv_wgrad_kernel<TP, true>), grid, dim3(256), lds, s, a);                         \
+    else hipLaunchKernelGGL((conv_wgrad_kernel<TP, false>), grid, dim3(256), lds, s, a);                            \
   } break;
   switch (p.TAPS) {
     XPT_WGRAD_CASE(1)
@@ -535,3 +693,43 @@
 #undef XPT_WGRAD_CASE
   return xpt_launch_status();
 }
+
+}
+
+extern "C" int xpt_conv2d_bwd_weight_partials(const void* g, const void* x, float* partials, size_t partial_floats, int B,
+                                              int PH, int PW, int C, int Cr, long long xpitch, int N, long long gpitch,
+                                              int KH, int KW, int stride, int pad_t, int pad_l, int OH, int OW,
+                                              int upsample, void* stream) {
+  return wgrad_launch(g, x, partials, partial_floats, B, PH, PW, C, Cr, xpitch, N, gpitch, KH, KW, stride, pad_t, pad_l, OH,
+                      OW, upsample, nullptr, stream);
+}
+
+extern "C" int xpt_conv2d_bwd_weight_act_blocks(int B, int PH, int PW, int C, int N, int KH, int KW, int stride, int pad_t,
+                                                int pad_l, int OH, int OW, int upsample) {
+  if (B <= 0 || PH <= 0 || PW <= 0 || C <= 0 || N <= 0 || KH <= 0 || KW <= 0 || stride <= 0 || OH <= 0 || OW <= 0)
+    return XPT_ERR_SHAPE;
+  if (C % 8 != 0 || N % 8 != 0 || (upsample != 0 && upsample != 1)) return 0;
+  if ((long long)B * OH * OW * N * 2 >= (1LL << 30)) return 0;
+  const int expect = xpt_conv2d_bwd_weight_splits(B, C, N, KH, KW, stride, OH, OW);
+  if (expect < 1) return 0;
+  constexpr int kMaxFoldBlocks = 3;
+  WfArgs f{};
+  if (fast_serves(B, PH, PW, C, N, KH, KW, stride, pad_t, pad_l, OH, OW, upsample, f))
+    return (f.ct <= kMaxFoldBlocks && fast_nsplit(f, N, C) == expect) ? expect : 0;
+  WgradPlan p;
+  if (!make_plan(B, C, N, KH, KW, stride, OH, OW, p)) return 0;
+  return ((C + 32 * p.WC - 1) / (32 * p.WC) <= kMaxFoldBlocks && p.nsplit == expect) ? expect : 0;
+}
+
+extern "C" int xpt_conv2d_bwd_weight_act_partials(const void* dy, long long dy_pitch, const void* y, float slope,
+                                                  const void* x, void* g_out, float* partials, size_t partial_floats,
+                                                  float* bias_partials, size_t bias_floats, int B, int PH, int PW, int C,
+                                                  int Cr, long long xpitch, int N, int KH, int KW, int stride, int pad_t,
+                                                  int pad_l, int OH, int OW, int upsample, void* stream) {
+  XPT_CHECK_PTR(dy); XPT_CHECK_PTR(g_out); XPT_CHECK_PTR(bias_partials);
+  if (slope != 1.f) XPT_CHECK_PTR(y);
+  if (!(slope >= 0.f) || ((uintptr_t)g_out) % 16 != 0 || (y && ((uintptr_t)y) % 16 != 0)) return XPT_ERR_ARG;
+  const ActFold act{slope != 1.f ? y : nullptr, g_out, bias_partials, bias_floats, slope};
+  return wgrad_launch(dy, x, partials, partial_floats, B, PH, PW, C, Cr, xpitch, N, dy_pitch, KH, KW, stride, pad_t, pad_l,
+                      OH, OW, upsample, &act, stream);
+}
diff --git a/xpt_mde_2021_amd/csrc/xpt_pointwise.hip b/xpt_mde_2021_amd/csrc/xpt_pointwise.hip
--- a/xpt_mde_2021_amd/csrc/xpt_pointwise.hip
+++ b/xpt_mde_2021_amd/csrc/xpt_pointwise.hip
@@ -112,7 +112,7 @@
         float yv[V];
         load_row<T, V>(y + o, yv);
 #pragma unroll
-        for (int i = 0; i < V; ++i) g[i] = yv[i] > 0.f ? g[i] : g[i] * slope;
+        for (int i = 0; i < V; ++i) g[i] = xpt_act_bwd(g[i], yv[i], slope);
       }
       if (need_dscale || relu_in) {
         load_row<T, V>(x + o, xv);
diff --git a/xpt_mde_2021_amd/hip/conv.py b/xpt_mde_2021_amd/hip/conv.py
--- a/xpt_mde_2021_amd/hip/conv.py
+++ b/xpt_mde_2021_amd/hip/conv.py
@@ -219,7 +219,12 @@
         rows = B * OH * OW
         dy, dpitch = _ops._rows_with_pitch(dy_in.to(_lib.half()))
         dbias = None
-        if ctx.has_bias or slope != 1.0:
+        fold = _fold_blocks(ctx, lib, dy, dpitch)
+        if fold:
+            g = torch.empty((B, N, OH, OW), dtype=_lib.half(), device=dy.device, memory_format=torch.channels_last)
+            _weight_grad_act(ctx, lib, dy, dpitch, y, g, x, fold)
+            gpitch = N
+        elif ctx.has_bias or slope != 1.0:
             g = torch.empty((B, N, OH, OW), dtype=_lib.half(), device=dy.device, memory_format=torch.channels_last)
             if ctx.sink_b is not None:
                 nblk = lib.xpt_affine_act_bwd_blocks(rows, N)
@@ -245,7 +250,7 @@
         if N % 8 != 0:
             raise _lib.XptHipError(f"conv backward: {N} output channels are not a multiple of 8")
         dx = dw = None
-        if ctx.needs_input_grad[1]:
+        if ctx.needs_input_grad[1] and not fold:
             if ctx.sink_w is not None and WGRAD_DEFER and getattr(weight, "defer_wgrad", False):
                 _deferred.append((ctx, g, gpitch, x))
                 side = None
@@ -314,6 +319,36 @@
     return _SIDE[device]
 
 
+WGRAD_FOLD_ACT = __import__("os").environ.get("XPT_WGRAD_FOLD_ACT", "1") == "1"
+
+
+def _fold_blocks(ctx, lib, dy, dpitch):
+    B, PH, PW, Cp, C, xpitch, N, KH, KW, stride, pt, pl, OH, OW, ups, slope = ctx.geom
+    if not WGRAD_FOLD_ACT or not (ctx.has_bias or slope != 1.0) or not ctx.needs_input_grad[1]:
+        return 0
+    if ctx.sink_w is None or (ctx.has_bias and ctx.sink_b is None) or WGRAD_SIDE_STREAM:
+        return 0
+    if WGRAD_DEFER and getattr(ctx.weight, "defer_wgrad", False):
+        return 0
+    if N % 8 != 0 or dpitch % 8 != 0 or dy.data_ptr() % 16 != 0:
+        return 0
+    return max(lib.xpt_conv2d_bwd_weight_act_blocks(B, PH, PW, Cp, N, KH, KW, stride, pt, pl, OH, OW, ups), 0)
+
+
+def _weight_grad_act(ctx, lib, dy, dpitch, y, g, x, nsplit):
+    B, PH, PW, Cp, C, xpitch, N, KH, KW, stride, pt, pl, OH, OW, ups, slope = ctx.geom
+    n = N * KH * KW * C
+    ws = _ops.grad_sink.partials(ctx.sink_w, "convw", nsplit * n)
+    wb = _ops.grad_sink.partials(ctx.sink_b if ctx.sink_b is not None else ctx.sink_w, "convw_bias", nsplit * 2 * N)
+    _lib.check(lib.xpt_conv2d_bwd_weight_act_partials(dy.data_ptr(), dpitch, None if y is None else y.data_ptr(), slope,
+                                                      x.data_ptr(), g.data_ptr(), ws.data_ptr(), ws.numel(), wb.data_ptr(),
+                                                      wb.numel(), B, PH, PW, Cp, C, xpitch, N, KH, KW, stride, pt, pl, OH,
+                                                      OW, ups, _stream()), "xpt_conv2d_bwd_weight_act_partials")
+    _ops.grad_sink.add(ctx.sink_w, ws, 0, n, nsplit, n)
+    if ctx.sink_b is not None:
+        _ops.grad_sink.add(ctx.sink_b, wb, 0, N, nsplit, 2 * N)
+
+
 def _weight_grad(ctx, lib, g, gpitch, x):
     B, PH, PW, Cp, C, xpitch, N, KH, KW, stride, pt, pl, OH, OW, ups, slope = ctx.geom
     nsplit = lib.xpt_conv2d_bwd_weight_splits(B, Cp, N, KH, KW, stride, OH, OW)
diff --git a/xpt_mde_2021_amd/hip/lib.py b/xpt_mde_2021_amd/hip/lib.py
--- a/xpt_mde_2021_amd/hip/lib.py
+++ b/xpt_mde_2021_amd/hip/lib.py
@@ -189,6 +189,9 @@
     "xpt_conv2d_bwd_weight_splits": (_i, [_i] * 8),
     "xpt_conv2d_bwd_weight_partials": (_i, [_p, _p, _p, _z, _i, _i, _i, _i, _i, ctypes.c_longlong, _i, ctypes.c_longlong,
                                             _i, _i, _i, _i, _i, _i, _i, _i, _p]),
+    "xpt_conv2d_bwd_weight_act_blocks": (_i, [_i] * 13),
+    "xpt_conv2d_bwd_weight_act_partials": (_i, [_p, ctypes.c_longlong, _p, _f, _p, _p, _p, _z, _p, _z, _i, _i, _i, _i, _i,
+                                                ctypes.c_longlong, _i, _i, _i, _i, _i, _i, _i, _i, _i, _p]),
     "xpt_headconv_bwd_blocks": (_i, [_i, _i, _i, _i]),
     "xpt_headconv_fwd": (_i, [_p, ctypes.c_longlong, _p, _p, _p, _i, _i, _i, _i, _p]),
     "xpt_headconv_bwd": (_i, [_p, ctypes.c_longlong, _p, _p, _p, _p, _z, _i, _i, _i, _i, _p]),
```
